# nverchev/PointCloudCounterfactual

Measured on AMD Instinct MI355X. Metric: clouds/sec Chamfer+EMD fwd+bwd, N=2048 B=32, higher is better.
Workload: dtype f32; 1 GPU; BASELINE configs[1]+[2]: N=2048 B=32 per GPU, nn_distance (Chamfer, mean) fwd+bwd + match_cost (approxmatch+matchcost) fwd+bwd through the autograd surface; inputs = "recon" clouds (reference permuted + N(0, 0.02^2): a trained autoencoder, SURVEY 8(d)); the 8(d) stress set (both clouds i.i.d. U[0,1]^3) is value_stress (--full); emd_mode=implicit, batch_per_gpu=32, n_points=2048, global_batch=32, parallelism=batch-sharded x1, no data-path collective, launcher=single process

## Files before the change

pointcloudcounterfactual_amd/backend.py:

```python

from __future__ import annotations

import ctypes

import torch

from pointcloudcounterfactual_amd import _lib
from pointcloudcounterfactual_amd._lib import call, ptr

_L = _lib.lib
F32, I32 = torch.float32, torch.int32


def _sizes(set_d: torch.Tensor, set_q: torch.Tensor) -> tuple[int, int, int]:
    return set_d.size(0), set_d.size(1), set_q.size(1)


def ApproxMatch(set_d: torch.Tensor, set_q: torch.Tensor) -> list[torch.Tensor]:
    b, n, m = _sizes(set_d, set_q)
    dev = set_d.device
    match = torch.empty((b, m, n), dtype=torch.float32, device=dev)
    temp = torch.empty((b, (n + m) * 2), dtype=torch.float32, device=dev)
    call(_L.pcc_approxmatch, 'ApproxMatch', dev, b, n, m, ptr(set_d, 'set_d', F32, dev), ptr(set_q, 'set_q', F32, dev),
         ptr(match, 'match', F32, dev), ptr(temp, 'temp', F32, dev))
    return [match, temp]


def ApproxMatchCost(set_d: torch.Tensor, set_q: torch.Tensor) -> list[torch.Tensor]:
    b, n, m = _sizes(set_d, set_q)
    dev = set_d.device
    match = torch.empty((b, m, n), dtype=torch.float32, device=dev)
    temp = torch.empty((b, (n + m) * 2), dtype=torch.float32, device=dev)
    cost = torch.empty((b,), dtype=torch.float32, device=dev)
    call(_L.pcc_approxmatch_cost, 'ApproxMatchCost', dev, b, n, m, ptr(set_d, 'set_d', F32, dev),
         ptr(set_q, 'set_q', F32, dev), ptr(match, 'match', F32, dev), ptr(temp, 'temp', F32, dev),
         ptr(cost, 'cost', F32, dev))
    return [match, temp, cost]


def MatchCostImplicit(set_d: torch.Tensor, set_q: torch.Tensor, with_grad: bool) -> list[torch.Tensor]:
    b, n, m = _sizes(set_d, set_q)
    dev = set_d.device
    cost = torch.empty((b,), dtype=torch.float32, device=dev)
    out = [cost]
    g1 = g2 = None
    if with_grad:
        g1 = torch.empty((b, n, 3), dtype=torch.float32, device=dev)
        g2 = torch.empty((b, m, 3), dtype=torch.float32, device=dev)
        out += [g1, g2]
    call(_L.pcc_match_cost, 'MatchCostImplicit', dev, b, n, m, ptr(set_d, 'set_d', F32, dev),
         ptr(set_q, 'set_q', F32, dev), None, ptr(cost, 'cost', F32, dev), ptr(g1, 'grad1', F32, dev),
         ptr(g2, 'grad2', F32, dev))
    return out


def MatchCost(set_d: torch.Tensor, set_q: torch.Tensor, match: torch.Tensor) -> torch.Tensor:
    b, n, m = _sizes(set_d, set_q)
    dev = set_d.device
    out = torch.empty((b,), dtype=torch.float32, device=dev)
    if match.numel() != b * n * m:
        raise RuntimeError(f'match has {match.numel()} elements, expected {b}x{m}x{n}')
    call(_L.pcc_matchcost, 'MatchCost', dev, b, n, m, ptr(set_d, 'set_d', F32, dev), ptr(set_q, 'set_q', F32, dev),
         ptr(match, 'match', F32, dev), ptr(out, 'cost', F32, dev))
    return out


def MatchCostGrad(set_d: torch.Tensor, set_q: torch.Tensor, match: torch.Tensor) -> list[torch.Tensor]:
    b, n, m = _sizes(set_d, set_q)
    dev = set_d.device
    grad1 = torch.empty((b, n, 3), dtype=torch.float32, device=dev)
    grad2 = torch.empty((b, m, 3), dtype=torch.float32, device=dev)
    if match.numel() != b * n * m:
        raise RuntimeError(f'match has {match.numel()} elements, expected {b}x{m}x{n}')
    call(_L.pcc_matchcostgrad, 'MatchCostGrad', dev, b, n, m, ptr(set_d, 'set_d', F32, dev),
         ptr(set_q, 'set_q', F32, dev), ptr(match, 'match', F32, dev), ptr(grad1, 'grad1', F32, dev),
         ptr(grad2, 'grad2', F32, dev))
    return [grad1, grad2]


def MatchCostGradScaled(set_d: torch.Tensor, set_q: torch.Tensor, match: torch.Tensor,
                        grad_cost: torch.Tensor) -> list[torch.Tensor]:
    b, n, m = _sizes(set_d, set_q)
    dev = set_d.device
    grad1 = torch.empty((b, n, 3), dtype=torch.float32, device=dev)
    grad2 = torch.empty((b, m, 3), dtype=torch.float32, device=dev)
    if match.numel() != b * n * m or grad_cost.numel() != b:
        raise RuntimeError('MatchCostGradScaled: match / grad_cost shapes do not match the clouds')
    call(_L.pcc_matchcostgrad_scaled, 'MatchCostGradScaled', dev, b, n, m, ptr(set_d, 'set_d', F32, dev),
         ptr(set_q, 'set_q', F32, dev), ptr(match, 'match', F32, dev), ptr(grad_cost, 'grad_cost', F32, dev),
         ptr(grad1, 'grad1', F32, dev), ptr(grad2, 'grad2', F32, dev))
    return [grad1, grad2]


def NNDistance(set_d: torch.Tensor, set_q: torch.Tensor) -> list[torch.Tensor]:
    b, n, m = _sizes(set_d, set_q)
    dev = set_d.device
    dist1 = torch.empty((b, n), dtype=torch.float32, device=dev)
    idx1 = torch.empty((b, n), dtype=torch.int32, device=dev)
    dist2 = torch.empty((b, m), dtype=torch.float32, device=dev)
    idx2 = torch.empty((b, m), dtype=torch.int32, device=dev)
    call(_L.pcc_nndistance, 'NNDistance', dev, b, n, ptr(set_d, 'set_d', F32, dev), m, ptr(set_q, 'set_q', F32, dev),
         ptr(dist1, 'dist1', F32, dev), ptr(idx1, 'idx1', I32, dev), ptr(dist2, 'dist2', F32, dev),
         ptr(idx2, 'idx2', I32, dev))
    return [dist1, idx1, dist2, idx2]


def ChamferLoss(set_d: torch.Tensor, set_q: torch.Tensor, mean: bool) -> list[torch.Tensor]:
    b, n, m = _sizes(set_d, set_q)
    dev = set_d.device
    loss = torch.empty((b,), dtype=torch.float32, device=dev)
    dist1 = torch.empty((b, n), dtype=torch.float32, device=dev)
    idx1 = torch.empty((b, n), dtype=torch.int32, device=dev)
    dist2 = torch.empty((b, m), dtype=torch.float32, device=dev)
    idx2 = torch.empty((b, m), dtype=torch.int32, device=dev)
    call(_L.pcc_chamfer_loss, 'ChamferLoss', dev, b, n, ptr(set_d, 'set_d', F32, dev), m, ptr(set_q, 'set_q', F32, dev),
         int(mean), ptr(loss, 'loss', F32, dev), ptr(dist1, 'dist1', F32, dev), ptr(idx1, 'idx1', I32, dev),
         ptr(dist2, 'dist2', F32, dev), ptr(idx2, 'idx2', I32, dev))
    return [loss, dist1, idx1, dist2, idx2]


def ChamferLossGrad(set_d: torch.Tensor, set_q: torch.Tensor, idx1: torch.Tensor, idx2: torch.Tensor,
                    grad_loss: torch.Tensor, mean: bool) -> list[torch.Tensor]:
    b, n, m = _sizes(set_d, set_q)
    dev = set_d.device
    grad1 = torch.empty((b, n, 3), dtype=torch.float32, device=dev)
    grad2 = torch.empty((b, m, 3), dtype=torch.float32, device=dev)
    if idx1.numel() != b * n or idx2.numel() != b * m or grad_loss.numel() != b:
        raise RuntimeError('ChamferLossGrad: idx / grad_loss shapes do not match the clouds')
    grad_loss, stride = _batch_stride(grad_loss, b)
    call(_L.pcc_chamfer_loss_grad, 'ChamferLossGrad', dev, b, n, ptr(set_d, 'set_d', F32, dev), m,
         ptr(set_q, 'set_q', F32, dev), ptr(idx1, 'idx1', I32, dev), ptr(idx2, 'idx2', I32, dev),
         ptr(grad_loss, 'grad_loss', F32, dev), stride, int(mean), ptr(grad1, 'grad1', F32, dev),
         ptr(grad2, 'grad2', F32, dev))
    return [grad1, grad2]


def ChamferEMD(set_d: torch.Tensor, set_q: torch.Tensor, mean: bool, with_grad: bool,
               return_dist: bool = False) -> list[torch.Tensor]:
    b, n, m = _sizes(set_d, set_q)
    dev = set_d.device
    loss = torch.empty((b,), dtype=torch.float32, device=dev)
    idx1 = torch.empty((b, n), dtype=torch.int32, device=dev)
    idx2 = torch.empty((b, m), dtype=torch.int32, device=dev)
    cost = torch.empty((b,), dtype=torch.float32, device=dev)
    out = [loss, idx1, idx2, cost]
    g1 = g2 = None
    if with_grad:
        g1 = torch.empty((b, n, 3), dtype=torch.float32, device=dev)
        g2 = torch.empty((b, m, 3), dtype=torch.float32, device=dev)
        out += [g1, g2]
    d1 = torch.empty((b, n), dtype=torch.float32, device=dev)
    d2 = torch.empty((b, m), dtype=torch.float32, device=dev)
    call(_L.pcc_chamfer_emd, 'ChamferEMD', dev, b, n, ptr(set_d, 'set_d', F32, dev), m, ptr(set_q, 'set_q', F32, dev),
         int(mean), ptr(loss, 'loss', F32, dev), ptr(d1, 'dist1', F32, dev), ptr(idx1, 'idx1', I32, dev),
         ptr(d2, 'dist2', F32, dev), ptr(idx2, 'idx2', I32, dev), ptr(cost, 'cost', F32, dev),
         ptr(g1, 'emd_grad1', F32, dev), ptr(g2, 'emd_grad2', F32, dev))
    if return_dist:
        out += [d1, d2]
    return out


def _batch_stride(g: torch.Tensor, b: int) -> tuple[torch.Tensor, int]:
    stride = g.stride(0) if g.dim() == 1 and b > 1 else 1
    if stride == 0:
        return g[:1], 0
    if stride != 1:
        return g.contiguous(), 1
    return g, 1


def ChamferEMDGrad(set_d: torch.Tensor, set_q: torch.Tensor, idx1: torch.Tensor, idx2: torch.Tensor,
                   grad_chamfer: torch.Tensor, mean: bool, emd_grad1: torch.Tensor, emd_grad2: torch.Tensor,
                   grad_emd: torch.Tensor) -> list[torch.Tensor]:
    b, n, m = _sizes(set_d, set_q)
    dev = set_d.device
    grad1 = torch.empty((b, n, 3), dtype=torch.float32, device=dev)
    grad2 = torch.empty((b, m, 3), dtype=torch.float32, device=dev)
    if (idx1.numel() != b * n or idx2.numel() != b * m or grad_chamfer.numel() != b or grad_emd.numel() != b
            or emd_grad1.numel() != b * n * 3 or emd_grad2.numel() != b * m * 3):
        raise RuntimeError('ChamferEMDGrad: shapes do not match the clouds')
    grad_chamfer, sc = _batch_stride(grad_chamfer, b)
    grad_emd, se = _batch_stride(grad_emd, b)
    call(_L.pcc_chamfer_emd_grad, 'ChamferEMDGrad', dev, b, n, ptr(set_d, 'set_d', F32, dev), m,
         ptr(set_q, 'set_q', F32, dev), ptr(idx1, 'idx1', I32, dev), ptr(idx2, 'idx2', I32, dev),
         ptr(grad_chamfer, 'grad_chamfer', F32, dev), sc, int(mean), ptr(emd_grad1, 'emd_grad1', F32, dev),
         ptr(emd_grad2, 'emd_grad2', F32, dev), ptr(grad_emd, 'grad_emd', F32, dev), se, ptr(grad1, 'grad1', F32, dev),
         ptr(grad2, 'grad2', F32, dev))
    return [grad1, grad2]


def NNDistanceGrad(set_d: torch.Tensor, set_q: torch.Tensor, idx1: torch.Tensor, idx2: torch.Tensor,
                   grad_dist1: torch.Tensor, grad_dist2: torch.Tensor) -> list[torch.Tensor]:
    b, n, m = _sizes(set_d, set_q)
    dev = set_d.device
    grad1 = torch.empty((b, n, 3), dtype=torch.float32, device=dev)
    grad2 = torch.empty((b, m, 3), dtype=torch.float32, device=dev)
    if idx1.numel() != b * n or grad_dist1.numel() != b * n or idx2.numel() != b * m or grad_dist2.numel() != b * m:
        raise RuntimeError('NNDistanceGrad: idx/grad_dist shapes do not match the clouds')
    call(_L.pcc_nndistancegrad, 'NNDistanceGrad', dev, b, n, ptr(set_d, 'set_d', F32, dev), m,
         ptr(set_q, 'set_q', F32, dev), ptr(grad_dist1, 'grad_dist1', F32, dev), ptr(idx1, 'idx1', I32, dev),
         ptr(grad_dist2, 'grad_dist2', F32, dev), ptr(idx2, 'idx2', I32, dev), ptr(grad1, 'grad1', F32, dev),
         ptr(grad2, 'grad2', F32, dev))
    return [grad1, grad2]


def SlicedWasserstein(set_d: torch.Tensor, set_q: torch.Tensor, theta: torch.Tensor, grad1: bool = False, grad2: bool = False,
                      per_direction: bool = False) -> list[torch.Tensor | None]:
    if set_d.dim() != 3 or set_d.size(2) != 3 or set_q.shape != set_d.shape:
        raise ValueError(f'SlicedWasserstein: clouds must be [B,N,3] of one shape, got {tuple(set_d.shape)} and {tuple(set_q.shape)}')
    if theta.dim() != 2 or theta.size(1) != 3:
        raise ValueError(f'SlicedWasserstein: directions must be [P,3], got {tuple(theta.shape)}')
    b, n, p = set_d.size(0), set_d.size(1), theta.size(0)
    dev = set_d.device
    cost = torch.empty((b,), dtype=torch.float32, device=dev)
    cost_p = torch.empty((b, p), dtype=torch.float32, device=dev) if per_direction else None
    g1 = torch.empty((b, n, 3), dtype=torch.float32, device=dev) if grad1 else None
    g2 = torch.empty((b, n, 3), dtype=torch.float32, device=dev) if grad2 else None
    call(_L.pcc_sliced_wasserstein, 'SlicedWasserstein', dev, b, n, p, ptr(set_d, 'set_d', F32, dev), ptr(set_q, 'set_q', F32, dev),
         ptr(theta, 'directions', F32, dev), ptr(cost, 'cost', F32, dev), ptr(cost_p, 'cost_p', F32, dev),
         ptr(g1, 'grad1', F32, dev), ptr(g2, 'grad2', F32, dev))
    return [cost, cost_p, g1, g2]


def Sinkhorn(set_d: torch.Tensor, set_q: torch.Tensor, eps: list[float], debias: bool = True, grad1: bool = False,
             grad2: bool = False, potentials: bool = False) -> list[torch.Tensor | None]:
    if set_d.dim() != 3 or set_q.dim() != 3 or set_d.size(2) != 3 or set_q.size(2) != 3 or set_d.size(0) != set_q.size(0):
        raise ValueError(f'Sinkhorn: clouds must be [B,N,3] and [B,M,3], got {tuple(set_d.shape)} and {tuple(set_q.shape)}')
    b, n, m = _sizes(set_d, set_q)
    dev = set_d.device
    sched = (ctypes.c_float * len(eps))(*eps)
    cost = torch.empty((b,), dtype=torch.float32, device=dev)
    p1 = torch.empty((b, n), dtype=torch.float32, device=dev) if potentials else None
    p2 = torch.empty((b, m), dtype=torch.float32, device=dev) if potentials else None
    g1 = torch.empty((b, n, 3), dtype=torch.float32, device=dev) if grad1 else None
    g2 = torch.empty((b, m, 3), dtype=torch.float32, device=dev) if grad2 else None
    call(_L.pcc_sinkhorn, 'Sinkhorn', dev, b, n, m, ptr(set_d, 'set_d', F32, dev), ptr(set_q, 'set_q', F32, dev), len(eps),
         ctypes.cast(sched, ctypes.c_void_p), int(bool(debias)), ptr(cost, 'cost', F32, dev), ptr(p1, 'pot1', F32, dev),
         ptr(p2, 'pot2', F32, dev), ptr(g1, 'grad1', F32, dev), ptr(g2, 'grad2', F32, dev))
    return [cost, p1, p2, g1, g2]
```

pointcloudcounterfactual_amd/csrc/am_pair.hip:

```cpp
#include "approxmatch.hpp"
#include "wave_ops.hpp"

#include <algorithm>

namespace {

using pcc::sq3;

constexpr int kPairRB = 8;
constexpr int kPairPad = 65;

struct PairArgs {
    int n, m, n4, m4;
    const float *soa1, *soa2;
    const float *lv;
    LevelConsts lc;
    float cut2[kLevels];
    float *cost_part;
    float *part1;
    float *part2;
    int col_blocks, row_tiles, bc;
};

template <int Q, bool GRAD>
__global__ __launch_bounds__(256) void am_pair_kernel(PairArgs a) {
    __shared__ float4 lds_l[kPairRT][3];
    __shared__ int lds_mask[kPairRT];
    __shared__ float stash[GRAD ? 4 * kPairRB * 3 * kPairPad : 4];
    __shared__ float lds_red[4];
    const int tid = threadIdx.x, lane = tid & 63;
    const int w = __builtin_amdgcn_readfirstlane(tid >> 6);
    const int cbn = a.col_blocks, rtn = a.row_tiles;
    const int item = (int)blockIdx.x / a.bc, smp = (int)blockIdx.x - item * a.bc;
    const int shift_k = item / cbn, cblk = item - shift_k * cbn;
    const int base_r = (int)(((long long)(2 * cblk + 1) * rtn) / (2 * cbn));
    const int shift = ((shift_k + 1) >> 1) * ((shift_k & 1) ? 1 : -1);
    const int rtile = ((base_r + shift) % rtn + rtn) % rtn;
    const int l0 = rtile * kPairRT;
    const int kb = cblk * 64 * Q;
    const int k0 = kb + lane * Q;
    const size_t nm4 = (size_t)a.n4 + a.m4;
    const float *lvb = a.lv + (size_t)smp * kLevels * nm4;
    const float *s1 = a.soa1 + (size_t)smp * 3 * a.n4;
    const float *s2 = a.soa2 + (size_t)smp * 3 * a.m4;
    const int lcnt = min(kPairRT, a.m - l0);

    float rowx = 0.f, rowy = 0.f, rowz = 0.f, rowr[kLevels];
#pragma unroll
    for (int i = 0; i < kLevels; i++) rowr[i] = 0.f;
    if (tid < lcnt) {
        const int l = l0 + tid;
        rowx = s2[l];
        rowy = s2[a.m4 + l];
        rowz = s2[2 * a.m4 + l];
#pragma unroll
        for (int i = 0; i < kLevels; i++) rowr[i] = lvb[(size_t)i * nm4 + a.n4 + l];
    }
    float x1[Q], y1[Q], z1[Q], rl[kLevels][Q];
    float blo[3] = {__builtin_inff(), __builtin_inff(), __builtin_inff()};
    float bhi[3] = {-__builtin_inff(), -__builtin_inff(), -__builtin_inff()};
#pragma unroll
    for (int q = 0; q < Q; q++) {
        const bool real = k0 + q < a.n;
        const int k = real ? k0 + q : a.n - 1;
        x1[q] = s1[k];
        y1[q] = s1[a.n4 + k];
        z1[q] = s1[2 * a.n4 + k];
#pragma unroll
        for (int i = 0; i < kLevels; i++) rl[i][q] = real ? lvb[(size_t)i * nm4 + k] : 0.f;
        blo[0] = fminf(blo[0], x1[q]); bhi[0] = fmaxf(bhi[0], x1[q]);
        blo[1] = fminf(blo[1], y1[q]); bhi[1] = fmaxf(bhi[1], y1[q]);
        blo[2] = fminf(blo[2], z1[q]); bhi[2] = fmaxf(bhi[2], z1[q]);
    }
#pragma unroll
    for (int c = 0; c < 3; c++) {
#pragma unroll
        for (int off = 1; off < 64; off <<= 1) {
            blo[c] = fminf(blo[c], __shfl_xor(blo[c], off, 64));
            bhi[c] = fmaxf(bhi[c], __shfl_xor(bhi[c], off, 64));
        }
    }
    if (tid < lcnt) {
        const float bx = fmaxf(fmaxf(blo[0] - rowx, rowx - bhi[0]), 0.f);
        const float by = fmaxf(fmaxf(blo[1] - rowy, rowy - bhi[1]), 0.f);
        const float bz = fmaxf(fmaxf(blo[2] - rowz, rowz - bhi[2]), 0.f);
        const float bd2 = bx * bx + by * by + bz * bz;
        int mask = 0;
#pragma unroll
        for (int i = 0; i < kLevels; i++) mask |= (rowr[i] != 0.f && !(bd2 > a.cut2[i])) ? (1 << i) : 0;
        lds_l[tid][0] = make_float4(rowx, rowy, rowz, rowr[0]);
        lds_l[tid][1] = make_float4(rowr[1], rowr[2], rowr[3], rowr[4]);
        lds_l[tid][2] = make_float4(rowr[5], rowr[6], rowr[7], rowr[8]);
        lds_mask[tid] = mask;
    }
    float g1[Q][3];
#pragma unroll
    for (int q = 0; q < Q; q++) g1[q][0] = g1[q][1] = g1[q][2] = 0.f;
    float csum = 0.f;
    float *my_stash = stash + (GRAD ? w * kPairRB * 3 * kPairPad : 0);
    __syncthreads();

    for (int base = 0; base < lcnt; base += 4 * kPairRB) {
#pragma unroll 1
        for (int s = 0; s < kPairRB; s++) {
            const int li = base + 4 * s + w;
            float rx = 0.f, ry = 0.f, rz = 0.f;
            const int mask = li < lcnt ? __builtin_amdgcn_readfirstlane(lds_mask[li]) : 0;
            if (mask) {
                const float4 A = lds_l[li][0], B = lds_l[li][1], Cc = lds_l[li][2];
                const float rr[kLevels] = {A.w, B.x, B.y, B.z, B.w, Cc.x, Cc.y, Cc.z, Cc.w};
                float ex[Q], ey[Q], ez[Q], d[Q], acc[Q];
#pragma unroll
                for (int q = 0; q < Q; q++) {
                    ex[q] = A.x - x1[q];
                    ey[q] = A.y - y1[q];
                    ez[q] = A.z - z1[q];
                    d[q] = sq3(ex[q], ey[q], ez[q]);
                    acc[q] = 0.f;
                }
#pragma unroll
                for (int i = 0; i < kLevels; i++) {
                    if (mask & (1 << i)) {
#pragma unroll
                        for (int q = 0; q < Q; q++)
                            acc[q] = __builtin_fmaf(fast_exp2(a.lc.c[i] * d[q]) * rl[i][q], rr[i], acc[q]);
                    }
                }
#pragma unroll
                for (int q = 0; q < Q; q++) {
                    if (GRAD) {
                        float dm;
                        asm("v_max_f32 %0, %1, %2" : "=v"(dm) : "v"(d[q]), "v"(1e-20f));
                        const float f = acc[q] * __builtin_amdgcn_rsqf(dm);
                        csum = __builtin_fmaf(f, d[q], csum);
                        g1[q][0] = __builtin_fmaf(-ex[q], f, g1[q][0]);
                        g1[q][1] = __builtin_fmaf(-ey[q], f, g1[q][1]);
                        g1[q][2] = __builtin_fmaf(-ez[q], f, g1[q][2]);
                        rx = __builtin_fmaf(ex[q], f, rx);
                        ry = __builtin_fmaf(ey[q], f, ry);
                        rz = __builtin_fmaf(ez[q], f, rz);
                    } else {
                        csum = __builtin_fmaf(acc[q], __builtin_amdgcn_sqrtf(d[q]), csum);
                    }
                }
            }
            if (GRAD) {
                my_stash[(s * 3 + 0) * kPairPad + lane] = rx;
                my_stash[(s * 3 + 1) * kPairPad + lane] = ry;
                my_stash[(s * 3 + 2) * kPairPad + lane] = rz;
            }
        }
        if (GRAD) {
            const int v = lane % 24, h = lane / 24;
            float t = 0.f;
            __builtin_amdgcn_wave_barrier();
            if (lane < 48) {
                const float *src = my_stash + v * kPairPad + h * 32;
#pragma unroll 8
                for (int i = 0; i < 32; i++) t += src[i];
            }
            __builtin_amdgcn_wave_barrier();
            const float hi = __shfl(t, lane + 24, 64);
            const int sl = v / 3, c = v - sl * 3;
            const int li = base + 4 * sl + w;
            if (lane < 24 && li < lcnt)
                a.part2[(((size_t)smp * cbn + cblk) * a.m4 + (l0 + li)) * 3 + c] = t + hi;
        }
    }
    csum = pcc::wave_sum_down(csum);
    if (lane == 0) lds_red[w] = csum;
    __syncthreads();
    if (tid == 0)
        a.cost_part[(size_t)smp * cbn * rtn + rtile * cbn + cblk] =
            ((lds_red[0] + lds_red[1]) + lds_red[2]) + lds_red[3];
    if (GRAD) {
        static_assert(Q * 3 * 64 <= 4 * kPairRB * 3 * kPairPad, "column merge reuses the stash");
        for (int src = 1; src < 4; src++) {
            __syncthreads();
            if (w == src) {
#pragma unroll
                for (int q = 0; q < Q; q++)
#pragma unroll
                    for (int c = 0; c < 3; c++) stash[(q * 3 + c) * 64 + lane] = g1[q][c];
            }
            __syncthreads();
            if (w == 0) {
#pragma unroll
                for (int q = 0; q < Q; q++)
#pragma unroll
                    for (int c = 0; c < 3; c++) g1[q][c] += stash[(q * 3 + c) * 64 + lane];
            }
        }
        if (w == 0) {
            float *dst = a.part1 + (((size_t)smp * rtn + rtile) * a.n4) * 3;
#pragma unroll
            for (int q = 0; q < Q; q++) {
                if (k0 + q < a.n) {
#pragma unroll
                    for (int c = 0; c < 3; c++) dst[(size_t)(k0 + q) * 3 + c] = g1[q][c];
                }
            }
        }
    }
}

struct FinishArgs {
    int parts[3], npts[2], pitch[2];
    const float *part[3];
    const int *perm[2];
    const float *scale;
    float *out[3];
    const float *ch_d1, *ch_d2;
    float *ch_loss;
    int ch_n, ch_m, ch_mean;
    const int *flags;
};
__global__ __launch_bounds__(256) void pair_finish_kernel(FinishArgs f) {
    __shared__ float red[256];
    const int which = blockIdx.z, smp = blockIdx.y, tid = threadIdx.x;
    if (which == 3) {
        if (blockIdx.x) return;
        __shared__ float red2[256];
        float s1 = 0.f, s2 = 0.f;
        auto strided_sum = [&](const float *d, int cnt) -> float {
            float acc = 0.f;
            for (int i0 = tid; i0 < cnt; i0 += 8 * 256) {
                float v[8];
#pragma unroll
                for (int u = 0; u < 8; u++) v[u] = d[min(i0 + u * 256, cnt - 1)];
#pragma unroll
                for (int u = 0; u < 8; u++)
                    if (i0 + u * 256 < cnt) acc += v[u];
            }
            return acc;
        };
        s1 = strided_sum(f.ch_d1 + (size_t)smp * f.ch_n, f.ch_n);
        s2 = strided_sum(f.ch_d2 + (size_t)smp * f.ch_m, f.ch_m);
        red[tid] = s1;
        red2[tid] = s2;
        __syncthreads();
        for (int off = 128; off > 0; off >>= 1) {
            if (tid < off) {
                red[tid] += red[tid + off];
                red2[tid] += red2[tid + off];
            }
            __syncthreads();
        }
        if (tid == 0) f.ch_loss[smp] = f.ch_mean ? red2[0] / (float)f.ch_m + red[0] / (float)f.ch_n : red[0] + red2[0];
        return;
    }
    const bool poisoned = f.flags && (f.flags[(size_t)smp * kLiveRow + kInfSlot] | f.flags[(size_t)smp * kLiveRow + kInfSlot + 1] |
                                      f.flags[(size_t)smp * kLiveRow + kErrSlot]);
    if (which == 2) {
        if (blockIdx.x) return;
        const int parts = f.parts[2];
        float s = 0.f;
        for (int i = tid; i < parts; i += 256) s += f.part[2][(size_t)smp * parts + i];
        red[tid] = s;
        __syncthreads();
        for (int off = 128; off > 0; off >>= 1) {
            if (tid < off) red[tid] += red[tid + off];
            __syncthreads();
        }
        if (tid == 0) f.out[2][smp] = poisoned ? __builtin_nanf("") : red[0];
        return;
    }
    if (!f.out[which]) return;
    const int npts = f.npts[which], pitch = f.pitch[which], parts = f.parts[which];
    const int i = blockIdx.x * 256 + tid;
    if (i >= npts * 3) return;
    const int s = i / 3, c = i - s * 3;
    const float *p = f.part[which] + (size_t)smp * parts * pitch * 3 + i;
    const int pt = f.perm[which][(size_t)smp * npts + s];
    const size_t stride = (size_t)pitch * 3;
    float acc = p[0];
    int t = 1;
    for (; t + 8 <= parts; t += 8) {
        float v[8];
#pragma unroll
        for (int u = 0; u < 8; u++) v[u] = p[(size_t)(t + u) * stride];
#pragma unroll
        for (int u = 0; u < 8; u++) acc += v[u];
    }
    {
        float v[7];
#pragma unroll
        for (int u = 0; u < 7; u++) v[u] = p[(size_t)min(t + u, parts - 1) * stride];
#pragma unroll
        for (int u = 0; u < 7; u++)
            if (t + u < parts) acc += v[u];
    }
    f.out[which][((size_t)smp * npts + pt) * 3 + c] = poisoned ? __builtin_nanf("") : f.scale ? acc * f.scale[smp] : acc;
}

template <int Q>
int launch_pair(const PairArgs &pa, dim3 grid, bool grad, hipStream_t st) {
    pcc::ProfScope prof(grad ? "am_pair_kernel<grad>" : "am_pair_kernel<cost>", st);
    if (grad) hipLaunchKernelGGL((am_pair_kernel<Q, true>), grid, dim3(256), 0, st, pa);
    else hipLaunchKernelGGL((am_pair_kernel<Q, false>), grid, dim3(256), 0, st, pa);
    return pcc::check_launch("match_cost(pair)");
}

}

namespace pcc {

int launch_pair_finish(const AmDims &L, const WsView &v, int s0, int bc, int col_blocks, int row_tiles, const float *grad_cost,
                       float *cost, float *grad1, float *grad2, const ChamferOut *chamfer, hipStream_t lst) {
    const size_t o = (size_t)s0;
    const int n = L.n, m = L.m;
    const bool grad = grad1 && grad2;
    const LevelConsts lc = make_levels();
    PairArgs pa{};
    pa.n = n; pa.m = m; pa.n4 = L.n4; pa.m4 = L.m4;
    pa.soa1 = v.soa1; pa.soa2 = v.soa2; pa.lv = v.lv;
    pa.lc = lc;
    for (int i = 0; i < kLevels; i++) pa.cut2[i] = zero_cut2(lc, i);
    pa.cost_part = v.pair_cost;
    pa.part1 = grad ? v.part1 : nullptr;
    pa.part2 = grad ? v.part2 : nullptr;
    pa.col_blocks = col_blocks; pa.row_tiles = row_tiles; pa.bc = bc;
    if ((long long)col_blocks * row_tiles * bc > 0x7fffffffLL) return pcc::invalid("match_cost: grid too large");
    const dim3 grid((unsigned)(col_blocks * row_tiles * bc));
    if (int rc = launch_pair<kPairQ>(pa, grid, grad, lst)) return rc;
    FinishArgs f{};
    f.parts[0] = row_tiles; f.parts[1] = col_blocks; f.parts[2] = col_blocks * row_tiles;
    f.npts[0] = n; f.npts[1] = m; f.pitch[0] = L.n4; f.pitch[1] = L.m4;
    f.part[0] = pa.part1; f.part[1] = pa.part2; f.part[2] = pa.cost_part;
    f.perm[0] = v.perm1; f.perm[1] = v.perm2;
    f.scale = grad_cost ? grad_cost + o : nullptr;
    f.out[0] = grad ? grad1 + o * n * 3 : nullptr;
    f.out[1] = grad ? grad2 + o * m * 3 : nullptr;
    f.out[2] = cost + o;
    f.flags = v.live_cnt;
    if (chamfer) {
        f.ch_d1 = chamfer->dist1 + o * n; f.ch_d2 = chamfer->dist2 + o * m; f.ch_loss = chamfer->loss + o;
        f.ch_n = n; f.ch_m = m; f.ch_mean = chamfer->mean;
    }
    {
        pcc::ProfScope prof("pair_finish_kernel", lst);
        const int blocks = grad ? pcc::ceil_div(std::max(n, m) * 3, 256) : 1;
        hipLaunchKernelGGL(pair_finish_kernel, dim3(blocks, bc, chamfer ? 4 : 3), dim3(256), 0, lst, f);
    }
    return pcc::check_launch("match_cost(reduce)");
}
}
```

pointcloudcounterfactual_amd/csrc/approxmatch.hip:

```cpp
#include "approxmatch.hpp"
#include "pcc_test_hooks.h"
#include "wave_ops.hpp"

#include <algorithm>
#include <functional>
#include <mutex>
#include <type_traits>

namespace {

using pcc::sq3;
using pcc::WsView;

enum Phase { PH_A = 0, PH_B = 1, PH_CA = 2, PH_C = 3 };

__device__ __forceinline__ float pass_a_ratio(float remL, float sum) { return remL / (1e-9f + sum); }
struct PassB {
    float ratio, remain;
};
__device__ __forceinline__ PassB pass_b(float remR, float sum) {
    const float sumr = sum * remR;
    const float consumption = __builtin_fminf(remR / (sumr + 1e-9f), 1.0f);
    return {consumption * remR, __builtin_fmaxf(0.0f, remR - sumr)};
}
__device__ __forceinline__ float pass_c_left(float remL, float ratioL, float sum) { return __builtin_fmaxf(0.0f, remL - ratioL * sum); }

struct PhaseArgs {
    int n_own, n_cand, tiles, batch;
    int own_n4, cand_n4, own_nb, cand_nb;
    const float *own_soa, *cand_soa;
    const float *cand_box;
    const float *own_box16;
    const float *w0, *w1;
    long long w0_stride, w1_stride;
    float w0c;
    float c0, c1;
    float cut2;
    float cut2_fine;
    int first;
    int level;
    float multiL, multiR;
    float *remain;
    float *remain_out;
    long long remain_stride;
    const float *ratio_in;
    float *ratio_out;
    long long ratio_stride;
    float *clist;
    int *clist_cnt;
    int cl_n4;
    const unsigned *mask_in;
    unsigned *mask_out;
    int mask_words;
    const int *live_in;
    int *live_out;
};

enum Var { V_PLAIN = 0, V_CULL = 1, V_COWN = 3, V_CLIST = 4 };

struct Sched {
    int n, m, n4, m4, nb1, nb2;
    const float *soa1, *soa2, *box1, *box2;
    float *rem, *lv;
    float multiL, multiR;
    float *clist;
    int *clist_cnt;
    int *live_cnt;
    unsigned *live_mask;
    int skip;
    LevelConsts lc;
};

inline int sched_phases() { return 2 * kLevels + 1; }

inline PhaseArgs build_phase(const Sched &sc, int p, int *mode_out, int *var_out) {
    const long long nm4 = (long long)sc.n4 + sc.m4;
    const long long rs = (long long)sc.n4 + 2LL * sc.m4;
    PhaseArgs a{};
    a.multiL = sc.multiL;
    a.multiR = sc.multiR;
    const bool set1_owns = (p == 0) || (p % 2 == 0);
    if (set1_owns) {
        a.n_own = sc.n; a.n_cand = sc.m; a.own_n4 = sc.n4; a.cand_n4 = sc.m4; a.own_nb = sc.nb1; a.cand_nb = sc.nb2;
        a.own_soa = sc.soa1; a.cand_soa = sc.soa2; a.cand_box = sc.box2;
        a.own_box16 = sc.box1;
    } else {
        a.n_own = sc.m; a.n_cand = sc.n; a.own_n4 = sc.m4; a.cand_n4 = sc.n4; a.own_nb = sc.nb2; a.cand_nb = sc.nb1;
        a.own_soa = sc.soa2; a.cand_soa = sc.soa1; a.cand_box = sc.box1;
        a.own_box16 = sc.box2;
    }
    int mode, var;
    if (p == 0) {
        mode = PH_A;
        var = sc.skip ? V_CULL : V_PLAIN;
        a.level = 0;
        a.w0 = nullptr; a.w0c = sc.multiR; a.c0 = sc.lc.c[0]; a.first = 1;
        a.cut2 = zero_cut2(sc.lc, 0);
        a.ratio_out = sc.lv; a.ratio_stride = kLevels * nm4;
    } else {
        const int i = (p - 1) / 2;
        float *ratioL = sc.lv + (size_t)i * nm4, *ratioR = ratioL + sc.n4;
        a.level = i;
        a.first = (i == 0);
        a.c0 = sc.lc.c[i];
        if (p % 2 == 1) {
            mode = PH_B;
            var = !sc.skip ? V_PLAIN : i <= 2 ? V_CULL : V_COWN;
            a.w0 = ratioL; a.w0_stride = kLevels * nm4;
            a.cut2 = zero_cut2(sc.lc, i);
            a.remain = sc.rem + sc.n4 + (i & 1) * sc.m4;
            a.remain_out = sc.rem + sc.n4 + ((i + 1) & 1) * sc.m4;
            a.remain_stride = rs;
            a.ratio_out = ratioR; a.ratio_stride = kLevels * nm4;
            if (var == V_COWN) { a.clist = sc.clist; a.clist_cnt = sc.clist_cnt; a.cl_n4 = sc.m4; }
            if (sc.live_mask) {
                const int words = mask_words(sc.m4);
                a.mask_words = words;
                if (i + 1 < kLevels && (var == V_COWN || i == 2)) a.mask_out = sc.live_mask + (size_t)(i + 1) * words;
                if (var == V_COWN) {
                    a.mask_in = sc.live_mask + (size_t)i * words;
                    a.remain = a.remain_out = sc.rem + sc.n4 + sc.m4;
                }
            }
            if (sc.live_cnt) {
                a.live_in = (var == V_COWN && i >= 1) ? sc.live_cnt + i : nullptr;
                a.live_out = i + 1 < kLevels ? sc.live_cnt + i + 1 : nullptr;
            }
        } else {
            mode = i + 1 < kLevels ? PH_CA : PH_C;
            var = !sc.skip ? V_PLAIN : i <= 2 ? V_CULL : V_CLIST;
            if (var == V_CLIST) { a.clist = sc.clist; a.clist_cnt = sc.clist_cnt; a.cl_n4 = sc.m4; }
            a.w0 = ratioR; a.w0_stride = kLevels * nm4;
            a.w1 = sc.rem + sc.n4 + ((i + 1) & 1) * sc.m4; a.w1_stride = rs;
            a.remain = sc.rem; a.remain_stride = rs;
            a.ratio_in = ratioL; a.ratio_stride = kLevels * nm4;
            const int lc_i = i + 1 < kLevels ? i + 1 : i;
            a.cut2 = zero_cut2(sc.lc, lc_i);
            a.cut2_fine = zero_cut2(sc.lc, i);
            if (i + 1 < kLevels) {
                a.c1 = sc.lc.c[i + 1];
                a.ratio_out = sc.lv + (size_t)(i + 1) * nm4;
            }
        }
    }
    *mode_out = mode;
    *var_out = var;
    return a;
}

template <int NW, int R, int S, int CH>
struct PhaseLds {
    static constexpr int kC = (3 + NW) * CH;
    static constexpr int kRed = NW * S * 64 * R;
    static constexpr int kOwn = 64 * R;
    static constexpr int kWave = S;
    static constexpr int floats = kC + kRed + kOwn + kWave + 4;
};

template <int MODE, int R, int S, int CH, int VAR, int G = 1>
__device__ __forceinline__ void am_phase_body(const PhaseArgs &a, int smp, int tile, float *smem) {
    constexpr int T = 64 * S;
    constexpr int TQ = 64 * R / G;
    constexpr int PQ = 64 * R;
    static_assert(G == 1 || (VAR == V_COWN && R == 1), "lane-split owners: owner-compacted launches only");
    constexpr int NW = (MODE == PH_CA) ? 2 : 1;
    constexpr bool W0_CONST = (MODE == PH_A);
    constexpr bool COWN = VAR == V_COWN, CLIST = VAR == V_CLIST;
    static_assert(VAR == V_PLAIN || COWN || CLIST, "the box-culled passes run on am_fine_kernel");
    static_assert(!(CLIST && W0_CONST), "pass A of the first level has constant weights");
    static_assert(TQ <= T, "one epilogue owner per thread");
    using L = PhaseLds<NW, R, S, CH>;
    float *lds_c = smem;
    float *red = smem + L::kC;
    int *own_idx = reinterpret_cast<int *>(red + L::kRed);
    int *wave_cnt = own_idx + L::kOwn;

    const int tid = threadIdx.x;
    const int lane = tid & 63;
    const int w = __builtin_amdgcn_readfirstlane(tid >> 6);
    const int sub = G > 1 ? lane / TQ : 0;
    const float *O = a.own_soa + (size_t)smp * 3 * a.own_n4;
    const float *C = a.cand_soa + (size_t)smp * 3 * a.cand_n4;
    const float *W0 = W0_CONST ? nullptr : a.w0 + (size_t)smp * a.w0_stride;
    const float *W1 = (NW == 2) ? a.w1 + (size_t)smp * a.w1_stride : nullptr;

    if (!COWN && tile * TQ >= a.n_own) return;
    static_assert(CH / 4 <= T, "one float4 group per thread and chunk");
    float4 st_x, st_y, st_z, st_0, st_1;
    auto stage_load = [&](const float *Cc, const float *W0c, const float *W1c, int pitch, int q0, int ngroups) {
        const int i = min(tid, max(ngroups - 1, 0));
        st_x = reinterpret_cast<const float4 *>(Cc + q0)[i];
        st_y = reinterpret_cast<const float4 *>(Cc + (size_t)pitch + q0)[i];
        st_z = reinterpret_cast<const float4 *>(Cc + (size_t)2 * pitch + q0)[i];
        st_0 = make_float4(a.w0c, a.w0c, a.w0c, a.w0c);
        st_1 = st_0;
        if (!W0_CONST) st_0 = *reinterpret_cast<const float4 *>(W0c + q0 + 4 * i);
        if (NW == 2) st_1 = *reinterpret_cast<const float4 *>(W1c + q0 + 4 * i);
    };
    if (COWN) stage_load(C, W0, W1, a.cand_n4, 0, (min(CH, a.n_cand) + 3) / 4);
    int n_valid = min(TQ, a.n_own - tile * TQ);
    if (COWN) {
        const int lo = tile * TQ, hi = lo + TQ;
        const unsigned *mk = a.mask_in + (size_t)smp * kLevels * a.mask_words;
        unsigned *mnext = (tile == 0 && a.mask_out) ? a.mask_out + (size_t)smp * kLevels * a.mask_words : nullptr;
        const int wpt = (a.mask_words + T - 1) / T;
        unsigned word = 0;
        int mine = 0;
        if (wpt == 1) {
            word = mk[min(tid, a.mask_words - 1)];
            word &= -(unsigned)(tid < a.mask_words);
            if (mnext && tid < a.mask_words) atomicAnd(&mnext[tid], word);
            mine = __popc(word);
        } else {
            for (int j = tid * wpt; j < min(tid * wpt + wpt, a.mask_words); j++) {
                const unsigned wj = mk[j];
                if (mnext) atomicAnd(&mnext[j], wj);
                mine += __popc(wj);
            }
        }
        int incl = mine;
#pragma unroll
        for (int off = 1; off < 64; off <<= 1) {
            const int v = __shfl_up(incl, off, 64);
            incl += lane >= off ? v : 0;
        }
        if (lane == 63) wave_cnt[w] = incl;
        __syncthreads();
        int before = 0, total = 0;
#pragma unroll
        for (int i = 0; i < S; i++) {
            const int c = __builtin_amdgcn_readfirstlane(wave_cnt[i]);
            before += i < w ? c : 0;
            total += c;
        }
        int pos = before + incl - mine - lo;
        auto deal = [&](unsigned bits, int first_owner) {
            while (bits) {
                const int bit = __builtin_ctz(bits);
                bits &= bits - 1;
                if ((unsigned)pos < (unsigned)TQ) own_idx[pos] = first_owner + bit;
                pos++;
            }
        };
        if (wpt == 1) {
            deal(word, tid * 32);
        } else {
            for (int j = tid * wpt; j < min(tid * wpt + wpt, a.mask_words); j++) deal(mk[j], j * 32);
        }
        if (a.clist_cnt && tile == 0 && tid == 0) a.clist_cnt[smp] = total;
        n_valid = min(TQ, total - lo);
        if (n_valid <= 0) return;
        (void)hi;
        __syncthreads();
    }
    int own_e = -1;
    if (tid < TQ && tid < n_valid) own_e = COWN ? own_idx[tid] : tile * TQ + tid;

    float ox[R], oy[R], oz[R], s0[R], s1[R];
    float t0x = 0.f, t1x = 0.f;
#pragma unroll
    for (int r = 0; r < R; r++) {
        const int e = G > 1 ? (lane & (TQ - 1)) : r * 64 + lane;
        int o = COWN ? own_idx[e < n_valid ? e : 0] : tile * TQ + e;
        o = o < a.n_own ? o : a.n_own - 1;
        ox[r] = O[o];
        oy[r] = O[a.own_n4 + o];
        oz[r] = O[2 * a.own_n4 + o];
        s0[r] = 0.f;
        s1[r] = 0.f;
    }
    float pre_rem = 0.f, pre_ratio = 0.f;
    {
        const int oe = max(own_e, 0);
        if (MODE != PH_A && !a.first) pre_rem = a.remain[(size_t)smp * a.remain_stride + oe];
        if (MODE == PH_CA || MODE == PH_C) pre_ratio = a.ratio_in[(size_t)smp * a.ratio_stride + oe];
    }
    const float4 *X4 = reinterpret_cast<const float4 *>(lds_c);
    const float4 *Y4 = X4 + CH / 4;
    const float4 *Z4 = Y4 + CH / 4;
    const float4 *A4 = Z4 + CH / 4;
    const float4 *B4 = A4 + CH / 4;
    const float c0 = a.c0, c1 = a.c1;

    const int n_cand = CLIST ? __builtin_amdgcn_readfirstlane(a.clist_cnt[smp]) : a.n_cand;
    if (CLIST) {
        C = a.clist + (size_t)smp * 5 * a.cl_n4;
        W0 = C + (size_t)3 * a.cl_n4;
        W1 = C + (size_t)4 * a.cl_n4;
    }
    const int cand_pitch = CLIST ? a.cl_n4 : a.cand_n4;
    for (int q0 = 0; q0 < n_cand; q0 += CH) {
        const int cnt = min(CH, n_cand - q0);
        int ngroups = (cnt + 3) / 4;
        if (q0) __syncthreads();
        {
            float4 *dst4 = reinterpret_cast<float4 *>(lds_c);
            if (!(COWN && q0 == 0)) stage_load(C, W0, W1, cand_pitch, q0, ngroups);
            const int i = tid;
            if (i < ngroups) {
                float4 vx = st_x, vy = st_y, vz = st_z, v0 = st_0, v1 = st_1;
                if (CLIST && i * 4 + 3 >= cnt) {
                    vx.y = i * 4 + 1 < cnt ? vx.y : 0.f; vx.z = i * 4 + 2 < cnt ? vx.z : 0.f; vx.w = 0.f;
                    vy.y = i * 4 + 1 < cnt ? vy.y : 0.f; vy.z = i * 4 + 2 < cnt ? vy.z : 0.f; vy.w = 0.f;
                    vz.y = i * 4 + 1 < cnt ? vz.y : 0.f; vz.z = i * 4 + 2 < cnt ? vz.z : 0.f; vz.w = 0.f;
                }
                if ((W0_CONST || CLIST) && i * 4 + 3 >= cnt) {
                    v0.x = i * 4 + 0 < cnt ? v0.x : 0.f;
                    v0.y = i * 4 + 1 < cnt ? v0.y : 0.f;
                    v0.z = i * 4 + 2 < cnt ? v0.z : 0.f;
                    v0.w = 0.f;
                    if (NW == 2) {
                        v1.x = i * 4 + 0 < cnt ? v1.x : 0.f;
                        v1.y = i * 4 + 1 < cnt ? v1.y : 0.f;
                        v1.z = i * 4 + 2 < cnt ? v1.z : 0.f;
                        v1.w = 0.f;
                    }
                }
                dst4[i] = vx;
                dst4[CH / 4 + i] = vy;
                dst4[2 * (CH / 4) + i] = vz;
                dst4[3 * (CH / 4) + i] = v0;
                if (NW == 2) dst4[4 * (CH / 4) + i] = v1;
            }
        }
        const int nblk = (ngroups + 3) / 4;
        __syncthreads();
        for (int blk = w; blk < nblk; blk += S) {
            const int g_end = min(blk * 4 + 4, ngroups);
            for (int g = blk * 4 + sub; g < g_end; g += G) {
                const float4 x = X4[g], y = Y4[g], z = Z4[g], wa = A4[g];
                float4 wb;
                if (NW == 2) wb = B4[g];
#pragma unroll
                for (int r = 0; r < R; r++) {
                    const float d0 = sq3(x.x - ox[r], y.x - oy[r], z.x - oz[r]);
                    const float d1 = sq3(x.y - ox[r], y.y - oy[r], z.y - oz[r]);
                    const float d2 = sq3(x.z - ox[r], y.z - oy[r], z.z - oz[r]);
                    const float d3 = sq3(x.w - ox[r], y.w - oy[r], z.w - oz[r]);
                    if (R == 1) {
                        s0[r] = __builtin_fmaf(fast_exp2(c0 * d0), wa.x, s0[r]);
                        t0x = __builtin_fmaf(fast_exp2(c0 * d1), wa.y, t0x);
                        s0[r] = __builtin_fmaf(fast_exp2(c0 * d2), wa.z, s0[r]);
                        t0x = __builtin_fmaf(fast_exp2(c0 * d3), wa.w, t0x);
                        if (NW == 2) {
                            s1[r] = __builtin_fmaf(fast_exp2(c1 * d0), wb.x, s1[r]);
                            t1x = __builtin_fmaf(fast_exp2(c1 * d1), wb.y, t1x);
                            s1[r] = __builtin_fmaf(fast_exp2(c1 * d2), wb.z, s1[r]);
                            t1x = __builtin_fmaf(fast_exp2(c1 * d3), wb.w, t1x);
                        }
                    } else {
                        s0[r] = __builtin_fmaf(fast_exp2(c0 * d0), wa.x, s0[r]);
                        s0[r] = __builtin_fmaf(fast_exp2(c0 * d1), wa.y, s0[r]);
                        s0[r] = __builtin_fmaf(fast_exp2(c0 * d2), wa.z, s0[r]);
                        s0[r] = __builtin_fmaf(fast_exp2(c0 * d3), wa.w, s0[r]);
                        if (NW == 2) {
                            s1[r] = __builtin_fmaf(fast_exp2(c1 * d0), wb.x, s1[r]);
                            s1[r] = __builtin_fmaf(fast_exp2(c1 * d1), wb.y, s1[r]);
                            s1[r] = __builtin_fmaf(fast_exp2(c1 * d2), wb.z, s1[r]);
                            s1[r] = __builtin_fmaf(fast_exp2(c1 * d3), wb.w, s1[r]);
                        }
                    }
                }
            }
        }
    }
    if (R == 1) {
        s0[0] += t0x;
        s1[0] += t1x;
    }
    if (G > 1) {
        s0[0] += __shfl_xor(s0[0], TQ, 64);
        if (G == 4) s0[0] += __shfl_xor(s0[0], 2 * TQ, 64);
    }
#pragma unroll
    for (int r = 0; r < R; r++) {
        red[(0 * S + w) * PQ + r * 64 + lane] = s0[r];
        if (NW == 2) red[(1 * S + w) * PQ + r * 64 + lane] = s1[r];
    }
    __syncthreads();
    if (own_e < 0) return;
    {
        const int e = tid;
        const int o = own_e;
        float t0 = red[e], t1 = 0.f;
        if (NW == 2) t1 = red[(1 * S) * PQ + e];
#pragma unroll
        for (int s = 1; s < S; s++) {
            t0 += red[(0 * S + s) * PQ + e];
            if (NW == 2) t1 += red[(1 * S + s) * PQ + e];
        }
        if (MODE == PH_A) {
            a.ratio_out[(size_t)smp * a.ratio_stride + o] = pass_a_ratio(a.multiL, t0);
        } else if (MODE == PH_B) {
            const PassB pb = pass_b(a.first ? a.multiR : pre_rem, t0);
            const float ratio_new = pb.ratio, remain_new = pb.remain;
            a.ratio_out[(size_t)smp * a.ratio_stride + o] = ratio_new;
            a.remain_out[(size_t)smp * a.remain_stride + o] = remain_new;
            if (a.live_out) {
                const unsigned long long alive = __ballot(remain_new != 0.f);
                if (lane == 0) atomicAdd(&a.live_out[(size_t)smp * kLiveRow], (int)__popcll(alive));
            }
            if (COWN && a.mask_out && remain_new == 0.f)
                atomicAnd(&a.mask_out[(size_t)smp * kLevels * a.mask_words + (o >> 5)], ~(1u << (o & 31)));
            if (COWN && a.clist) {
                float cx = ox[0], cy = oy[0], cz = oz[0];
#pragma unroll
                for (int r = 1; r < R; r++) {
                    cx = w == r ? ox[r] : cx;
                    cy = w == r ? oy[r] : cy;
                    cz = w == r ? oz[r] : cz;
                }
                float *cl = a.clist + (size_t)smp * 5 * a.cl_n4 + tile * TQ + e;
                cl[0] = cx;
                cl[(size_t)a.cl_n4] = cy;
                cl[(size_t)2 * a.cl_n4] = cz;
                cl[(size_t)3 * a.cl_n4] = ratio_new;
                cl[(size_t)4 * a.cl_n4] = remain_new;
            }
        } else {
            const float left = pass_c_left(a.first ? a.multiL : pre_rem, pre_ratio, t0);
            a.remain[(size_t)smp * a.remain_stride + o] = left;
            if (MODE == PH_CA) a.ratio_out[(size_t)smp * a.ratio_stride + o] = pass_a_ratio(left, t1);
        }
    }
}

template <int MODE, int R, int S, int CH, int VAR, int G = 1>
__global__ __launch_bounds__(64 * S) void am_phase_kernel(PhaseArgs a) {
    __shared__ __attribute__((aligned(16))) float smem[PhaseLds<(MODE == PH_CA ? 2 : 1), R, S, CH>::floats];
    constexpr bool COWN = VAR == V_COWN;
    int smp, tile;
    const int bid = (int)blockIdx.x, nwg = (int)gridDim.x;
    if (COWN) {
        if (a.batch % 8 == 0) {
            const int per = a.batch / 8, i = bid / 8;
            smp = (bid % 8) + 8 * (i % per);
            tile = i / per;
        } else {
            smp = bid % a.batch;
            tile = bid / a.batch;
        }
        if (a.live_in && tile > 0 && tile * (64 * R / G) >= a.live_in[(size_t)smp * kLiveRow]) return;
    } else {
        const int lid = pcc::xcd_contiguous(bid, nwg);
        smp = lid / a.tiles;
        tile = lid - smp * a.tiles;
    }
    am_phase_body<MODE, R, S, CH, VAR, G>(a, smp, tile, smem);
}

constexpr int kFineS = 8;
constexpr int kFineOG = 16;
constexpr int kFineGroups = 64 / kFineOG;
constexpr int kFineQ = 4;

struct FineOwners {
    float x[kFineQ], y[kFineQ], z[kFineQ];
};
struct FineRows {
    const float *x, *y, *z, *w0, *w1;
};

__device__ __forceinline__ void fine_group_box(const float *own_box, int own_nb, int smp, int g16, float4 &lo, float4 &hi) {
    lo = make_float4(__builtin_inff(), __builtin_inff(), __builtin_inff(), 0.f);
    hi = make_float4(-__builtin_inff(), -__builtin_inff(), -__builtin_inff(), 0.f);
    if (g16 < own_nb) {
        const float4 *ob = reinterpret_cast<const float4 *>(own_box + ((size_t)smp * own_nb + g16) * 8);
        lo = ob[0];
        hi = ob[1];
    }
}

__device__ __forceinline__ float fine_box_d2(const float4 &glo, const float4 &ghi, const float *cand_box) {
    const float4 *cb = reinterpret_cast<const float4 *>(cand_box);
    const float4 lo = cb[0], hi = cb[1];
    const float dx = fmaxf(fmaxf(glo.x - hi.x, lo.x - ghi.x), 0.f);
    const float dy = fmaxf(fmaxf(glo.y - hi.y, lo.y - ghi.y), 0.f);
    const float dz = fmaxf(fmaxf(glo.z - hi.z, lo.z - ghi.z), 0.f);
    return dx * dx + dy * dy + dz * dz;
}

template <int NBLK>
__device__ __forceinline__ void fine_block_list(bool keep, bool outer_only, int tid, int tg, int tb, int w, int lane,
                                                int *wave_cnt, unsigned char (*items)[NBLK], unsigned char *need) {
    if (tid < NBLK) need[tid] = 0;
    const unsigned long long bal = __ballot(keep);
    if (lane == 0) wave_cnt[w] = __popcll(bal);
    __syncthreads();
    const int before = (w & 1) ? wave_cnt[w - 1] : 0;
    if (keep) {
        items[tg][before + __popcll(bal & ((1ull << lane) - 1ull))] = (unsigned char)(tb | (outer_only ? 128 : 0));
        need[tb] = 1;
    }
    __syncthreads();
}

template <int NW>
__device__ __forceinline__ void fine_walk(const FineRows &rows, const unsigned char *list, int nitems, int cs, int cl, float c0,
                                          float c1, const FineOwners &own, float (&s0)[kFineQ], float (&s1)[kFineQ]) {
    for (int it = cs; it < nitems; it += 2) {
        const int item = __builtin_amdgcn_readfirstlane((int)list[it]);
        const int ci = (item & 127) * kBox + cl;
        const float x = rows.x[ci], y = rows.y[ci], z = rows.z[ci];
        if (NW == 2 && (item & 128)) {
            const float wb = rows.w1[ci];
#pragma unroll
            for (int j = 0; j < kFineQ; j++) s1[j] = __builtin_fmaf(fast_exp2(c1 * sq3(x - own.x[j], y - own.y[j], z - own.z[j])), wb, s1[j]);
            continue;
        }
        const float wa = rows.w0[ci];
        float wb = 0.f;
        if (NW == 2) wb = rows.w1[ci];
#pragma unroll
        for (int j = 0; j < kFineQ; j++) {
            const float d = sq3(x - own.x[j], y - own.y[j], z - own.z[j]);
            s0[j] = __builtin_fmaf(fast_exp2(c0 * d), wa, s0[j]);
            if (NW == 2) s1[j] = __builtin_fmaf(fast_exp2(c1 * d), wb, s1[j]);
        }
    }
}

template <int NW>
__device__ __forceinline__ void fine_reduce(float (&s0)[kFineQ], float (&s1)[kFineQ], float (*red)[2][64], int cs, int cl, int og, int quad) {
    const auto add = [](float a, float b) { return a + b; };
#pragma unroll
    for (int j = 0; j < kFineQ; j++) {
        s0[j] = pcc::row_reduce16(s0[j], add);
        if (NW == 2) s1[j] = pcc::row_reduce16(s1[j], add);
    }
    if (cl == 0) {
#pragma unroll
        for (int j = 0; j < kFineQ; j++) {
            red[0][cs][og * kFineOG + quad * kFineQ + j] = s0[j];
            if (NW == 2) red[1][cs][og * kFineOG + quad * kFineQ + j] = s1[j];
        }
    }
}

template <int MODE, int CH>
__global__ __launch_bounds__(64 * kFineS, MODE == PH_CA ? 4 : 8) void am_fine_kernel(PhaseArgs a) {
    constexpr int T = 64 * kFineS;
    constexpr int NW = (MODE == PH_CA) ? 2 : 1;
    constexpr bool W0_CONST = (MODE == PH_A);
    constexpr int NBLK = CH / kBox;
    static_assert(kFineGroups * NBLK == T, "one (owner group, candidate block) box test per thread");
    static_assert(kFineOG == kBox && kFineOG * kFineQ == 64, "a wave = 16 candidates x 4 owner quads");
    __shared__ __attribute__((aligned(16))) float lds_c[(3 + NW) * CH];
    __shared__ float red[NW][2][64];
    __shared__ unsigned char items[kFineGroups][NBLK];
    __shared__ unsigned char need[NBLK];
    __shared__ int wave_cnt[kFineS];

    const int lid = pcc::xcd_contiguous((int)blockIdx.x, (int)gridDim.x);
    const int smp = lid / a.tiles;
    const int tile = lid - smp * a.tiles;
    const int tid = threadIdx.x, lane = tid & 63;
    const int w = __builtin_amdgcn_readfirstlane(tid >> 6);
    const int og = w & (kFineGroups - 1);
    const int cs = w / kFineGroups;
    const int cl = lane & (kBox - 1);
    const int quad = lane / kBox;
    const float *O = a.own_soa + (size_t)smp * 3 * a.own_n4;
    const float *C = a.cand_soa + (size_t)smp * 3 * a.cand_n4;
    const float *W0 = W0_CONST ? nullptr : a.w0 + (size_t)smp * a.w0_stride;
    const float *W1 = (NW == 2) ? a.w1 + (size_t)smp * a.w1_stride : nullptr;

    FineOwners own;
    float s0[kFineQ], s1[kFineQ];
#pragma unroll
    for (int j = 0; j < kFineQ; j++) {
        int o = tile * 64 + og * kFineOG + quad * kFineQ + j;
        o = o < a.n_own ? o : a.n_own - 1;
        own.x[j] = O[o];
        own.y[j] = O[a.own_n4 + o];
        own.z[j] = O[2 * a.own_n4 + o];
        s0[j] = 0.f;
        s1[j] = 0.f;
    }
    const int own_e = (tid < 64 && tile * 64 + tid < a.n_own) ? tile * 64 + tid : -1;
    float pre_rem = 0.f, pre_ratio = 0.f;
    {
        const int oe = max(own_e, 0);
        if (MODE != PH_A && !a.first) pre_rem = a.remain[(size_t)smp * a.remain_stride + oe];
        if (MODE == PH_CA || MODE == PH_C) pre_ratio = a.ratio_in[(size_t)smp * a.ratio_stride + oe];
    }
    const int tg = tid / NBLK, tb = tid - tg * NBLK;
    float4 glo, ghi;
    fine_group_box(a.own_box16, a.own_nb, smp, tile * kFineGroups + tg, glo, ghi);
    const float c0 = a.c0, c1 = a.c1, cut2 = a.cut2;
    const FineRows rows = {lds_c, lds_c + CH, lds_c + 2 * CH, lds_c + 3 * CH, lds_c + 4 * CH};

    for (int q0 = 0; q0 < a.n_cand; q0 += CH) {
        const int cnt = min(CH, a.n_cand - q0);
        const int ngroups = (cnt + 3) / 4;
        const int nblk = (ngroups + 3) / 4;
        if (q0) __syncthreads();
        bool keep = false, outer_only = false;
        if (tb < nblk) {
            const float bd2 = fine_box_d2(glo, ghi, a.cand_box + ((size_t)smp * a.cand_nb + q0 / kBox + tb) * 8);
            keep = !(bd2 > cut2);
            outer_only = NW == 2 && bd2 > a.cut2_fine;
        }
        fine_block_list<NBLK>(keep, outer_only, tid, tg, tb, w, lane, wave_cnt, items, need);
        {
            float4 *dst4 = reinterpret_cast<float4 *>(lds_c);
            const float4 *sx = reinterpret_cast<const float4 *>(C + q0);
            const float4 *sy = reinterpret_cast<const float4 *>(C + (size_t)a.cand_n4 + q0);
            const float4 *sz = reinterpret_cast<const float4 *>(C + (size_t)2 * a.cand_n4 + q0);
            static_assert(CH / 4 <= T, "one float4 group per thread and chunk");
            const int i = tid;
            if (i < nblk * 4 && need[i >> 2]) {
                float4 vx = make_float4(0.f, 0.f, 0.f, 0.f), vy = vx, vz = vx, v0 = vx, v1 = vx;
                if (i < ngroups) {
                    vx = sx[i]; vy = sy[i]; vz = sz[i];
                    v0 = W0_CONST ? make_float4(a.w0c, a.w0c, a.w0c, a.w0c) : *reinterpret_cast<const float4 *>(W0 + q0 + 4 * i);
                    if (NW == 2) v1 = *reinterpret_cast<const float4 *>(W1 + q0 + 4 * i);
                    if (W0_CONST && i * 4 + 3 >= cnt) {
                        v0.x = i * 4 + 0 < cnt ? v0.x : 0.f;
                        v0.y = i * 4 + 1 < cnt ? v0.y : 0.f;
                        v0.z = i * 4 + 2 < cnt ? v0.z : 0.f;
                        v0.w = 0.f;
                    }
                }
                dst4[i] = vx;
                dst4[CH / 4 + i] = vy;
                dst4[2 * (CH / 4) + i] = vz;
                dst4[3 * (CH / 4) + i] = v0;
                if (NW == 2) dst4[4 * (CH / 4) + i] = v1;
            }
        }
        __syncthreads();
        fine_walk<NW>(rows, items[og], wave_cnt[2 * og] + wave_cnt[2 * og + 1], cs, cl, c0, c1, own, s0, s1);
    }
    fine_reduce<NW>(s0, s1, red, cs, cl, og, quad);
    __syncthreads();
    if (own_e < 0) return;
    const float sum0 = red[0][0][tid] + red[0][1][tid];
    const float sum1 = NW == 2 ? red[NW - 1][0][tid] + red[NW - 1][1][tid] : 0.f;
    if (MODE == PH_A) {
        a.ratio_out[(size_t)smp * a.ratio_stride + own_e] = pass_a_ratio(a.multiL, sum0);
    } else if (MODE == PH_B) {
        const PassB pb = pass_b(a.first ? a.multiR : pre_rem, sum0);
        a.ratio_out[(size_t)smp * a.ratio_stride + own_e] = pb.ratio;
        a.remain_out[(size_t)smp * a.remain_stride + own_e] = pb.remain;
        if (a.live_out) {
            const unsigned long long alive = __ballot(pb.remain != 0.f);
            if (lane == 0) atomicAdd(&a.live_out[(size_t)smp * kLiveRow], (int)__popcll(alive));
            if (a.mask_out && lane == 0) {
                unsigned *mo = a.mask_out + (size_t)smp * kLevels * a.mask_words;
                if (2 * tile < a.mask_words) mo[2 * tile] = (unsigned)alive;
                if (2 * tile + 1 < a.mask_words) mo[2 * tile + 1] = (unsigned)(alive >> 32);
            }
        }
    } else {
        const float left = pass_c_left(a.first ? a.multiL : pre_rem, pre_ratio, sum0);
        a.remain[(size_t)smp * a.remain_stride + own_e] = left;
        if (MODE == PH_CA) a.ratio_out[(size_t)smp * a.ratio_stride + own_e] = pass_a_ratio(left, sum1);
    }
}

constexpr int kFpPasses = 7;
constexpr int kFpCH = 2048;

struct FinePersistArgs {
    int n, m, n4, m4, nb1, nb2, tiles;
    const float *soa1, *soa2, *box1, *box2;
    float *rem, *lv;
    float multiL, multiR;
    float c[4], cut2[4];
    int *live_cnt;
    unsigned *live_mask;
    int mask_words;
    unsigned *host_err;
    int inject;
};

__global__ __launch_bounds__(64 * kFineS) void am_fine_persist_kernel(FinePersistArgs a) {
    constexpr int T = 64 * kFineS, CH = kFpCH, NBLK = CH / kBox;
    static_assert(kFineGroups * NBLK == T, "one (owner group, candidate block) box test per thread and direction");
    __shared__ __attribute__((aligned(16))) float lds_p[2][3 * CH];
    __shared__ __attribute__((aligned(16))) float lds_w[2][CH];
    __shared__ float red[2][2][64];
    __shared__ unsigned char items[kFineGroups][NBLK];
    __shared__ unsigned char need[NBLK];
    __shared__ int wave_cnt[kFineS];

    const int lid = pcc::xcd_contiguous((int)blockIdx.x, (int)gridDim.x);
    const int smp = lid / a.tiles;
    const int tile = lid - smp * a.tiles;
    const int tid = threadIdx.x, lane = tid & 63;
    const int w = __builtin_amdgcn_readfirstlane(tid >> 6);
    const int og = w & (kFineGroups - 1), cs = w / kFineGroups;
    const int cl = lane & (kBox - 1), quad = lane / kBox;
    const long long nm4 = (long long)a.n4 + a.m4, rs = (long long)a.n4 + 2LL * a.m4;
    const float *S1 = a.soa1 + (size_t)smp * 3 * a.n4;
    const float *S2 = a.soa2 + (size_t)smp * 3 * a.m4;
    float *LV = a.lv + (size_t)smp * kLevels * nm4;
    float *REM = a.rem + (size_t)smp * rs;
    int *row = a.live_cnt + (size_t)smp * kLiveRow;
    unsigned *bar = reinterpret_cast<unsigned *>(row + kBarSlot);
    unsigned *err = reinterpret_cast<unsigned *>(row + kErrSlot);

    for (int s = 0; s < 2; s++) {
        const float *S = s ? S2 : S1;
        const int p4 = s ? a.m4 : a.n4, ngroups = p4 / 4, nblk = (ngroups + 3) / 4;
        float4 *dst4 = reinterpret_cast<float4 *>(lds_p[s]);
        const float4 *sx = reinterpret_cast<const float4 *>(S);
        const float4 *sy = reinterpret_cast<const float4 *>(S + p4);
        const float4 *sz = reinterpret_cast<const float4 *>(S + 2 * (size_t)p4);
        for (int i = tid; i < nblk * 4; i += T) {
            float4 vx = make_float4(0.f, 0.f, 0.f, 0.f), vy = vx, vz = vx;
            if (i < ngroups) { vx = sx[i]; vy = sy[i]; vz = sz[i]; }
            dst4[i] = vx;
            dst4[CH / 4 + i] = vy;
            dst4[2 * (CH / 4) + i] = vz;
        }
    }
    FineOwners set1, set2;
#pragma unroll
    for (int j = 0; j < kFineQ; j++) {
        const int o = tile * 64 + og * kFineOG + quad * kFineQ + j;
        const int o1 = min(o, a.n - 1), o2 = min(o, a.m - 1);
        set1.x[j] = S1[o1]; set1.y[j] = S1[a.n4 + o1]; set1.z[j] = S1[2 * a.n4 + o1];
        set2.x[j] = S2[o2]; set2.y[j] = S2[a.m4 + o2]; set2.z[j] = S2[2 * a.m4 + o2];
    }
    const int tg = tid / NBLK, tb = tid - tg * NBLK;
    auto box_d2 = [&](const float *own_box, int own_nb, const float *cand_box, int cand_nb) -> float {
        float4 glo, ghi;
        fine_group_box(own_box, own_nb, smp, tile * kFineGroups + tg, glo, ghi);
        if (tb >= cand_nb) return __builtin_inff();
        return fine_box_d2(glo, ghi, cand_box + ((size_t)smp * cand_nb + tb) * 8);
    };
    const float d2_role0 = box_d2(a.box1, a.nb1, a.box2, a.nb2);
    const float d2_role1 = box_d2(a.box2, a.nb2, a.box1, a.nb1);
    const int own1 = (tid < 64 && tile * 64 + tid < a.n) ? tile * 64 + tid : -1;
    const int own2 = (tid < 64 && tile * 64 + tid < a.m) ? tile * 64 + tid : -1;
    float remL = 0.f, ratL = 0.f, remR = 0.f;
    unsigned arrivals = 0;
    bool ok = true;

    auto pass = [&](auto mode_tag, int i) {
        constexpr int MODE = decltype(mode_tag)::value;
        constexpr int NW = MODE == PH_CA ? 2 : 1;
        constexpr int ROLE = MODE == PH_B ? 1 : 0;
        const int n_cand = ROLE ? a.n : a.m, cand_n4 = ROLE ? a.n4 : a.m4;
        const int nblk = (cand_n4 / 4 + 3) / 4;
        const float c0 = a.c[i], c1 = a.c[MODE == PH_CA ? i + 1 : i];
        const float cut2 = a.cut2[MODE == PH_CA ? i + 1 : i];
        const float *P = lds_p[ROLE ? 0 : 1];
        const float bd2 = ROLE ? d2_role1 : d2_role0;
        const bool keep = tb < nblk && !(bd2 > cut2);
        const bool outer_only = NW == 2 && bd2 > a.cut2[i];
        fine_block_list<NBLK>(keep, outer_only, tid, tg, tb, w, lane, wave_cnt, items, need);
        {
            const float *W0 = MODE == PH_A ? nullptr : MODE == PH_B ? LV + (size_t)i * nm4 : LV + (size_t)i * nm4 + a.n4;
            const float *W1 = MODE == PH_CA ? REM + a.n4 + (size_t)((i + 1) & 1) * a.m4 : nullptr;
            for (int idx = tid; idx < nblk * kBox; idx += T) {
                if (!need[idx >> 4]) continue;
                float v0, v1 = 0.f;
                if (MODE == PH_A) v0 = idx < n_cand ? a.multiR : 0.f;
                else v0 = idx < cand_n4 ? pcc::agent_ld(W0 + idx) : 0.f;
                if (NW == 2) v1 = idx < cand_n4 ? pcc::agent_ld(W1 + idx) : 0.f;
                lds_w[0][idx] = v0;
                if (NW == 2) lds_w[1][idx] = v1;
            }
        }
        __syncthreads();
        float s0[kFineQ], s1[kFineQ];
#pragma unroll
        for (int j = 0; j < kFineQ; j++) s0[j] = s1[j] = 0.f;
        const FineRows rows = {P, P + CH, P + 2 * CH, lds_w[0], lds_w[1]};
        fine_walk<NW>(rows, items[og], wave_cnt[2 * og] + wave_cnt[2 * og + 1], cs, cl, c0, c1, ROLE ? set2 : set1, s0, s1);
        fine_reduce<NW>(s0, s1, red, cs, cl, og, quad);
        __syncthreads();
        const int own_e = ROLE ? own2 : own1;
        if (own_e >= 0) {
            const float sum0 = red[0][0][tid] + red[0][1][tid];
            const float sum1 = NW == 2 ? red[1][0][tid] + red[1][1][tid] : 0.f;
            if (MODE == PH_A) {
                ratL = pass_a_ratio(a.multiL, sum0);
                pcc::agent_st(LV + own_e, ratL);
            } else if (MODE == PH_B) {
                const PassB pb = pass_b(i == 0 ? a.multiR : remR, sum0);
                pcc::agent_st(LV + (size_t)i * nm4 + a.n4 + own_e, pb.ratio);
                pcc::agent_st(REM + a.n4 + (size_t)((i + 1) & 1) * a.m4 + own_e, pb.remain);
                remR = pb.remain;
                if (i == 2) {
                    const unsigned long long alive = __ballot(pb.remain != 0.f);
                    if (lane == 0) {
                        atomicAdd(&row[3], (int)__popcll(alive));
                        unsigned *mo = a.live_mask + ((size_t)smp * kLevels + 3) * a.mask_words;
                        if (2 * tile < a.mask_words) mo[2 * tile] = (unsigned)alive;
                        if (2 * tile + 1 < a.mask_words) mo[2 * tile + 1] = (unsigned)(alive >> 32);
                    }
                }
            } else {
                remL = pass_c_left(i == 0 ? a.multiL : remL, ratL, sum0);
                pcc::agent_st(REM + own_e, remL);
                ratL = pass_a_ratio(remL, sum1);
                pcc::agent_st(LV + (size_t)(i + 1) * nm4 + own_e, ratL);
            }
        }
    };
    auto barrier = [&]() -> bool {
        arrivals += (unsigned)a.tiles;
        return pcc::coresident_barrier<1, (1u << 22)>(bar, arrivals, err, a.host_err, [&] {
            const unsigned seen = pcc::agent_ld(bar);
            return 1u | ((arrivals / (unsigned)a.tiles) << 4) | ((seen & 0xfffu) << 8) | ((unsigned)smp << 20);
        });
    };
    if (a.inject && tile == 0 && tid == 0) pcc::coresident_fail(err, a.host_err, 1u | ((unsigned)smp << 20));
    __syncthreads();
    pass(std::integral_constant<int, PH_A>{}, 0);
    for (int i = 0; i < 3 && ok; i++) {
        ok = barrier();
        if (!ok) break;
        pass(std::integral_constant<int, PH_B>{}, i);
        ok = barrier();
        if (!ok) break;
        pass(std::integral_constant<int, PH_CA>{}, i);
    }
}

__global__ __launch_bounds__(256) void am_unpermute_kernel(int n, int m, int n4, int m4,
                                                            const float *__restrict__ lv_sorted,
                                                            const float *__restrict__ rem_sorted,
                                                            const int *__restrict__ rank1,
                                                            const int *__restrict__ rank2,
                                                            const int *__restrict__ flags,
                                                            float *__restrict__ lv, float *__restrict__ temp) {
    const int smp = blockIdx.y;
    const int i = blockIdx.x * 256 + threadIdx.x;
    if (i >= n + m) return;
    const int s = i < n ? rank1[(size_t)smp * n + i] : n4 + rank2[(size_t)smp * m + (i - n)];
    const size_t nm = (size_t)n + m, nm4 = (size_t)n4 + m4;
    const float *src = lv_sorted + (size_t)smp * kLevels * nm4;
    float *dst = lv + (size_t)smp * kLevels * nm;
    const bool failed = flags[(size_t)smp * kLiveRow + kErrSlot] != 0;
    float last = 0.f;
#pragma unroll
    for (int l = 0; l < kLevels; l++) {
        last = failed ? __builtin_nanf("") : src[(size_t)l * nm4 + s];
        dst[(size_t)l * nm + i] = last;
    }
    float *tb = temp + (size_t)smp * 2 * nm;
    tb[i] = failed ? __builtin_nanf("") : rem_sorted[(size_t)smp * (nm4 + m4) + (i < n ? s : s + m4)];
    tb[nm + i] = last;
}

constexpr int kMatLT = 64;
constexpr int kMatKT = 256;

template <bool COST, bool VEC>
__global__ __launch_bounds__(256) void am_materialise_kernel(int n, int m, const float *__restrict__ xyz1,
                                                              const float *__restrict__ xyz2,
                                                              const float *__restrict__ lv, LevelConsts lc,
                                                              float *__restrict__ match,
                                                              float *__restrict__ cost_part) {
    __shared__ float4 lds_l[kMatLT][3];
    __shared__ float lds_red[4];
    const int tid = threadIdx.x, lane = tid & 63;
    const int w = __builtin_amdgcn_readfirstlane(tid >> 6);
    const int smp = blockIdx.z;
    const int l0 = blockIdx.y * kMatLT;
    const int k0 = blockIdx.x * kMatKT + lane * 4;
    const size_t lvs = (size_t)kLevels * (n + m);
    const float *lvb = lv + (size_t)smp * lvs;
    const float *p1 = xyz1 + (size_t)smp * n * 3;
    const float *p2 = xyz2 + (size_t)smp * m * 3;
    const int lcnt = min(kMatLT, m - l0);

    if (tid < lcnt) {
        const int l = l0 + tid;
        float rr[kLevels];
#pragma unroll
        for (int i = 0; i < kLevels; i++) rr[i] = lvb[(size_t)i * (n + m) + n + l];
        lds_l[tid][0] = make_float4(p2[l * 3 + 0], p2[l * 3 + 1], p2[l * 3 + 2], rr[0]);
        lds_l[tid][1] = make_float4(rr[1], rr[2], rr[3], rr[4]);
        lds_l[tid][2] = make_float4(rr[5], rr[6], rr[7], rr[8]);
    }
    float x1[4], y1[4], z1[4], rl[kLevels][4];
#pragma unroll
    for (int q = 0; q < 4; q++) {
        int k = k0 + q;
        k = k < n ? k : n - 1;
        x1[q] = p1[k * 3 + 0];
        y1[q] = p1[k * 3 + 1];
        z1[q] = p1[k * 3 + 2];
#pragma unroll
        for (int i = 0; i < kLevels; i++) rl[i][q] = lvb[(size_t)i * (n + m) + k];
    }
    __syncthreads();
    float csum = 0.f;
    for (int li = w; li < lcnt; li += 4) {
        const float4 A = lds_l[li][0], B = lds_l[li][1], Cc = lds_l[li][2];
        const float rr[kLevels] = {A.w, B.x, B.y, B.z, B.w, Cc.x, Cc.y, Cc.z, Cc.w};
        int live[kLevels];
#pragma unroll
        for (int i = 0; i < kLevels; i++) live[i] = __builtin_amdgcn_readfirstlane((int)(rr[i] != 0.f));
        float d[4], acc[4];
#pragma unroll
        for (int q = 0; q < 4; q++) {
            d[q] = sq3(A.x - x1[q], A.y - y1[q], A.z - z1[q]);
            acc[q] = 0.f;
        }
#pragma unroll
        for (int i = 0; i < kLevels; i++) {
            if (live[i]) {
#pragma unroll
                for (int q = 0; q < 4; q++) acc[q] += (fast_exp2(lc.c[i] * d[q]) * rl[i][q]) * rr[i];
            }
        }
        float out[4];
#pragma unroll
        for (int q = 0; q < 4; q++) {
            out[q] = acc[q];
            if (COST && k0 + q < n) csum = __builtin_fmaf(acc[q], __builtin_amdgcn_sqrtf(d[q]), csum);
        }
        float *row = match + ((size_t)smp * m + (l0 + li)) * n;
        if (VEC) {
            if (k0 + 3 < n) {
                v4f o4 = {out[0], out[1], out[2], out[3]};
                __builtin_nontemporal_store(o4, reinterpret_cast<v4f *>(row + k0));
            } else {
#pragma unroll
                for (int q = 0; q < 4; q++)
                    if (k0 + q < n) row[k0 + q] = out[q];
            }
        } else {
#pragma unroll
            for (int q = 0; q < 4; q++)
                if (k0 + q < n) row[k0 + q] = out[q];
        }
    }
    if (COST) {
        csum = pcc::wave_sum_down(csum);
        if (lane == 0) lds_red[w] = csum;
        __syncthreads();
        if (tid == 0)
            cost_part[(size_t)smp * gridDim.x * gridDim.y + blockIdx.y * gridDim.x + blockIdx.x] =
                ((lds_red[0] + lds_red[1]) + lds_red[2]) + lds_red[3];
    }
}

constexpr int kPhCH = 2048;
constexpr int kClistCH = 1024;

static bool cull_enabled() {
    return pcc::tuning(PCC_TUNE_AM_NOCULL) == 0;
}

template <int MODE>
const char *phase_name(int level, bool skipping) {
    static const char *const names[4][kLevels][2] = {
        {{"am_phase_kernel<A> L0 plain", "am_phase_kernel<A> L0 fine"}, {"", ""}, {"", ""}, {"", ""}, {"", ""},
         {"", ""}, {"", ""}, {"", ""}, {"", ""}},
        {{"am_phase_kernel<B> L0 plain", "am_phase_kernel<B> L0 fine"},
         {"am_phase_kernel<B> L1 plain", "am_phase_kernel<B> L1 fine"},
         {"am_phase_kernel<B> L2 plain", "am_phase_kernel<B> L2 fine"},
         {"am_phase_kernel<B> L3 plain", "am_phase_kernel<B> L3 own"},
         {"am_phase_kernel<B> L4 plain", "am_phase_kernel<B> L4 own"},
         {"am_phase_kernel<B> L5 plain", "am_phase_kernel<B> L5 own"},
         {"am_phase_kernel<B> L6 plain", "am_phase_kernel<B> L6 own"},
         {"am_phase_kernel<B> L7 plain", "am_phase_kernel<B> L7 own"},
         {"am_phase_kernel<B> L8 plain", "am_phase_kernel<B> L8 own"}},
        {{"am_phase_kernel<CA> L0 plain", "am_phase_kernel<CA> L0 fine"},
         {"am_phase_kernel<CA> L1 plain", "am_phase_kernel<CA> L1 fine"},
         {"am_phase_kernel<CA> L2 plain", "am_phase_kernel<CA> L2 fine"},
         {"am_phase_kernel<CA> L3 plain", "am_phase_kernel<CA> L3 list"},
         {"am_phase_kernel<CA> L4 plain", "am_phase_kernel<CA> L4 list"},
         {"am_phase_kernel<CA> L5 plain", "am_phase_kernel<CA> L5 list"},
         {"am_phase_kernel<CA> L6 plain", "am_phase_kernel<CA> L6 list"},
         {"am_phase_kernel<CA> L7 plain", "am_phase_kernel<CA> L7 list"}, {"", ""}},
        {{"", ""}, {"", ""}, {"", ""}, {"", ""}, {"", ""}, {"", ""}, {"", ""}, {"", ""},
         {"am_phase_kernel<C> L8 plain", "am_phase_kernel<C> L8 list"}}};
    return names[MODE][level][skipping];
}

template <int MODE, int R, int S, int G = 1>
int launch_phase_rs(PhaseArgs a, int b, int var, hipStream_t st, const char *what) {
    a.tiles = pcc::ceil_div(a.n_own, 64 * R / G);
    a.batch = b;
    const long long grid = (long long)b * a.tiles;
    if (grid > 0x7fffffffLL) return pcc::invalid("approxmatch: grid too large");
    {
        const bool skipping = (var == V_CLIST && (MODE == PH_CA || MODE == PH_C)) || (var == V_COWN && MODE == PH_B);
        pcc::ProfScope prof(phase_name<MODE>(a.level, skipping), st);
        const dim3 g((unsigned)grid), blk(64 * S);
        if (var == V_CLIST && (MODE == PH_CA || MODE == PH_C))
            hipLaunchKernelGGL((am_phase_kernel<(MODE == PH_CA || MODE == PH_C) ? MODE : PH_C, R, S, kClistCH, V_CLIST>), g, blk, 0, st, a);
        else if (var == V_COWN && MODE == PH_B)
            hipLaunchKernelGGL((am_phase_kernel<PH_B, (G > 1 ? 1 : R), S, kPhCH, V_COWN, G>), g, blk, 0, st, a);
        else hipLaunchKernelGGL((am_phase_kernel<MODE, R, S, kPhCH, V_PLAIN>), g, blk, 0, st, a);
    }
    return pcc::check_launch(what);
}

template <int MODE>
int launch_fine(PhaseArgs a, int b, hipStream_t st, const char *what) {
    a.tiles = pcc::ceil_div(a.n_own, 64);
    a.batch = b;
    const long long grid = (long long)b * a.tiles;
    if (grid > 0x7fffffffLL) return pcc::invalid("approxmatch: grid too large");
    {
        pcc::ProfScope prof(phase_name<MODE>(a.level, true), st);
        hipLaunchKernelGGL((am_fine_kernel<(MODE == PH_C ? PH_CA : MODE), kPhCH>), dim3((unsigned)grid), dim3(64 * kFineS), 0, st, a);
    }
    return pcc::check_launch(what);
}

template <int MODE>
int launch_phase(const PhaseArgs &a, int b, int var, hipStream_t st, const char *what) {
    if (var == V_CULL) return launch_fine<MODE>(a, b, st, what);
    if (var == V_COWN) {
        if (a.live_in && a.level >= 5) return launch_phase_rs<MODE, 1, 8, 4>(a, b, var, st, what);
        if (a.live_in && a.level >= 4) return launch_phase_rs<MODE, 1, 8, 2>(a, b, var, st, what);
        return launch_phase_rs<MODE, 1, 8>(a, b, var, st, what);
    }
    const long long owners = (long long)b * a.n_own;
    if (var == V_CLIST && owners < 4LL * 65536) return launch_phase_rs<MODE, 1, 8>(a, b, var, st, what);
    if (owners >= 4LL * 65536) return launch_phase_rs<MODE, 4, 8>(a, b, var, st, what);
    if (owners >= 32768) return launch_phase_rs<MODE, 2, 8>(a, b, var, st, what);
    return launch_phase_rs<MODE, 1, 8>(a, b, var, st, what);
}

size_t cost_parts(int n, int m) { return (size_t)pcc::ceil_div(n, kMatKT) * pcc::ceil_div(m, kMatLT); }

struct WsLayout : pcc::AmDims {
    int b;
    int col_blocks, row_tiles;
    bool grad;
    size_t total;
    WsLayout(int b_, int n_, int m_, int col_blocks_ = 0, int row_tiles_ = 0, bool grad_ = false)
        : AmDims(n_, m_), b(b_), col_blocks(col_blocks_), row_tiles(row_tiles_), grad(grad_) {
        WsView unused;
        total = carve(0, 0, unused);
    }
    WsView view(char *base, int s) const {
        WsView v;
        carve(reinterpret_cast<uintptr_t>(base), (size_t)s, v);
        return v;
    }

  private:
    size_t carve(uintptr_t base, size_t s, WsView &v) const {
        size_t o = 0;
        auto sec = [&](auto *&p, size_t per) {
            using T = std::remove_reference_t<decltype(*p)>;
            p = reinterpret_cast<T *>(base + o + s * per * sizeof(T));
            o = (o + (size_t)b * per * sizeof(T) + 15) & ~(size_t)15;
        };
        sec(v.soa1, 3 * (size_t)n4);
        sec(v.soa2, 3 * (size_t)m4);
        sec(v.rank1, n);
        sec(v.rank2, m);
        sec(v.perm1, n);
        sec(v.perm2, m);
        sec(v.box1, (size_t)nb1 * 8);
        sec(v.box2, (size_t)nb2 * 8);
        sec(v.rem, rem_floats());
        sec(v.lv, lv_floats());
        sec(v.lv_orig, kLevels * ((size_t)n + m));
        sec(v.cpart, cost_parts(n, m));
        sec(v.clist, 5 * (size_t)m4);
        sec(v.clist_cnt, 1);
        sec(v.live_cnt, kLiveRow);
        sec(v.live_mask, (size_t)kLevels * mask_words(m4));
        sec(v.aos1, n);
        sec(v.aos2, m);
        sec(v.pair_cost, (size_t)col_blocks * row_tiles);
        sec(v.part1, grad ? (size_t)row_tiles * n4 * 3 : 0);
        sec(v.part2, grad ? (size_t)col_blocks * m4 * 3 : 0);
        return o;
    }
};

constexpr int kMaxLanes = 2;
hipStream_t side_stream() {
    static std::mutex mu;
    static hipStream_t streams[64] = {};
    int dev = 0;
    if (hipGetDevice(&dev) != hipSuccess || dev < 0 || dev >= 64) return nullptr;
    std::lock_guard<std::mutex> lk(mu);
    if (!streams[dev]) {
        int least = 0, greatest = 0;
        if (hipDeviceGetStreamPriorityRange(&least, &greatest) != hipSuccess) {
            (void)hipGetLastError();
            least = greatest = 0;
        }
        if (hipStreamCreateWithPriority(&streams[dev], hipStreamNonBlocking, greatest) != hipSuccess) {
            (void)hipGetLastError();
            if (hipStreamCreateWithFlags(&streams[dev], hipStreamNonBlocking) != hipSuccess) {
                streams[dev] = nullptr;
                (void)hipGetLastError();
            }
        }
    }
    return streams[dev];
}

struct ForkJoin {
    hipStream_t main, side = nullptr;
    ForkJoin(hipStream_t m, bool fork) : main(m) {
        if (!fork) return;
        hipEvent_t ev;
        if (hipEventCreateWithFlags(&ev, hipEventDisableTiming) != hipSuccess) return;
        if (hipEventRecord(ev, main) == hipSuccess) {
            hipStream_t s = side_stream();
            if (s && hipStreamWaitEvent(s, ev, 0) == hipSuccess) side = s;
        }
        (void)hipEventDestroy(ev);
    }
    ~ForkJoin() {
        if (!side) return;
        hipEvent_t ev;
        if (hipEventCreateWithFlags(&ev, hipEventDisableTiming) != hipSuccess) {
            (void)hipStreamSynchronize(side);
            return;
        }
        (void)hipEventRecord(ev, side);
        (void)hipStreamWaitEvent(main, ev, 0);
        (void)hipEventDestroy(ev);
    }
};

static bool resident_enabled() {
    return pcc::tuning(PCC_TUNE_AM_NORESIDENT) == 0;
}
int launch_fine_resident(const Sched &sc, int bc, hipStream_t st) {
    if (!sc.skip || !sc.live_cnt || !sc.live_mask || !resident_enabled()) return -1;
    if (sc.n > kFpCH || sc.m > kFpCH || sc.n < 1 || sc.m < 1) return -1;
    const int tiles = pcc::ceil_div(std::max(sc.n, sc.m), 64);
    FinePersistArgs a{};
    a.n = sc.n; a.m = sc.m; a.n4 = sc.n4; a.m4 = sc.m4; a.nb1 = sc.nb1; a.nb2 = sc.nb2; a.tiles = tiles;
    a.soa1 = sc.soa1; a.soa2 = sc.soa2; a.box1 = sc.box1; a.box2 = sc.box2;
    a.rem = sc.rem; a.lv = sc.lv; a.multiL = sc.multiL; a.multiR = sc.multiR;
    for (int i = 0; i < 4; i++) {
        a.c[i] = sc.lc.c[i];
        a.cut2[i] = zero_cut2(sc.lc, i);
    }
    a.live_cnt = sc.live_cnt;
    a.live_mask = sc.live_mask;
    a.mask_words = mask_words(sc.m4);
    static const int per_cu = [] {
        int r = 0;
        const void *k = reinterpret_cast<const void *>(am_fine_persist_kernel);
        if (hipOccupancyMaxActiveBlocksPerMultiprocessor(&r, k, 64 * kFineS, 0) != hipSuccess) (void)hipGetLastError();
        return r;
    }();
    if (per_cu < 2 || (long long)bc * tiles > pcc::device_cus()) return -1;
    pcc::CoresidentGate gate(pcc::kFineResident, st);
    if (!gate.ok) return -1;
    a.host_err = gate.sticky;
    a.inject = gate.inject;
    {
        pcc::ProfScope prof("am_fine_persist_kernel", st);
        hipLaunchKernelGGL(am_fine_persist_kernel, dim3((unsigned)(bc * tiles)), dim3(64 * kFineS), 0, st, a);
    }
    return pcc::check_launch("approxmatch(resident fine levels)");
}

Sched lane_sched(const WsLayout &L, const WsView &v, const LevelConsts &lc) {
    Sched sc{};
    sc.n = L.n; sc.m = L.m; sc.n4 = L.n4; sc.m4 = L.m4; sc.nb1 = L.nb1; sc.nb2 = L.nb2;
    sc.soa1 = v.soa1; sc.soa2 = v.soa2; sc.box1 = v.box1; sc.box2 = v.box2; sc.rem = v.rem; sc.lv = v.lv;
    if (L.n >= L.m) { sc.multiL = 1; sc.multiR = (float)(L.n / L.m); }
    else { sc.multiL = (float)(L.m / L.n); sc.multiR = 1; }
    sc.skip = cull_enabled() ? 1 : 0;
    sc.lc = lc;
    sc.clist = v.clist; sc.clist_cnt = v.clist_cnt;
    if (sc.skip) { sc.live_cnt = v.live_cnt; sc.live_mask = v.live_mask; }
    return sc;
}

int run_levels(const WsLayout &L, char *base, const float *xyz1, const float *xyz2, const LevelConsts &lc, hipStream_t st,
               const std::function<int(int, int, hipStream_t)> &lane_tail = nullptr,
               const std::function<int(int, int, hipStream_t)> &after_sort = nullptr) {
    if (const unsigned fw = pcc::take_coresident_failure(pcc::kFineResident)) {
        char buf[320];
        std::snprintf(buf, sizeof buf, "approxmatch: an earlier call on this device did not complete (a sample barrier of the resident "
                      "fine-level launch timed out: barrier %u of sample %u saw %u arrivals; the implicit path reported NaN for those "
                      "samples); this call was not started", (fw >> 4) & 0xfu, fw >> 20, (fw >> 8) & 0xfffu);
        return pcc::invalid(buf);
    }
    const bool split_enabled = pcc::tuning(PCC_TUNE_AM_NOSPLIT) == 0;

    struct Lane {
        int s0, bc;
        hipStream_t st;
        WsView v;
        Sched sc;
    };
    Lane lanes[kMaxLanes];
    int nlanes = 1;
    bool fork = false;
    if (split_enabled && L.b >= 8 && (long long)L.b * std::max(L.n, L.m) >= 32768) {
        fork = !pcc::capturing(st);
    }
    ForkJoin fj(st, fork);
    if (fj.side) nlanes = 2;
    for (int l = 0; l < nlanes; l++) {
        Lane &ln = lanes[l];
        ln.s0 = (int)((long long)L.b * l / nlanes);
        ln.bc = (int)((long long)L.b * (l + 1) / nlanes) - ln.s0;
        ln.st = l == 0 ? st : fj.side;
        ln.v = L.view(base, ln.s0);
        ln.sc = lane_sched(L, ln.v, lc);
    }
    int rc = PCC_OK;
    auto enqueue_head = [&](int l) -> int {
        const Lane &ln = lanes[l];
        const size_t s0 = (size_t)ln.s0;
        int r = pcc::sort_clouds(L, ln.v, ln.bc, xyz1 + s0 * L.n * 3, xyz2 + s0 * L.m * 3, (bool)after_sort, ln.st);
        if (!r && after_sort && l % 2 == 0) r = after_sort(ln.s0, ln.bc, ln.st);
        return r;
    };
    auto enqueue_pass = [&](int l, int p) -> int {
        const Lane &ln = lanes[l];
        int mode, var;
        const PhaseArgs a = build_phase(ln.sc, p, &mode, &var);
        switch (mode) {
        case PH_A: return launch_phase<PH_A>(a, ln.bc, var, ln.st, "approxmatch(A)");
        case PH_B: return launch_phase<PH_B>(a, ln.bc, var, ln.st, "approxmatch(B)");
        case PH_CA: return launch_phase<PH_CA>(a, ln.bc, var, ln.st, "approxmatch(CA)");
        default: return launch_phase<PH_C>(a, ln.bc, var, ln.st, "approxmatch(C)");
        }
    };
    int first_pass[kMaxLanes] = {};
    {
        for (int l = 0; l < nlanes && !rc; l++) rc = enqueue_head(l);
        if (rc) return rc;
        {
            pcc::ProfScope seq0("am_phase_sequence", lanes[0].st, true);
            pcc::ProfScope seq1("am_phase_sequence", lanes[nlanes > 1 ? 1 : 0].st, true, nlanes >= 2);
            for (int l = 0; l < nlanes && !rc; l++) {
                const int r = launch_fine_resident(lanes[l].sc, lanes[l].bc, lanes[l].st);
                if (r > 0) rc = r;
                else if (r == 0) first_pass[l] = kFpPasses;
            }
            for (int p = 0; p < sched_phases() && !rc; p++)
                for (int l = 0; l < nlanes && !rc; l++)
                    if (p >= first_pass[l]) rc = enqueue_pass(l, p);
            if (rc) return rc;
        }
        if (after_sort)
            for (int l = 1; l < nlanes; l += 2)
                if (int rc2 = after_sort(lanes[l].s0, lanes[l].bc, lanes[l].st)) return rc2;
        if (lane_tail) {
            for (int l = 0; l < nlanes; l++)
                if (int rc2 = lane_tail(lanes[l].s0, lanes[l].bc, lanes[l].st)) return rc2;
        }
    }
    return PCC_OK;
}

int approxmatch_impl(int b, int n, int m, const float *xyz1, const float *xyz2, float *match, float *temp,
                     void *workspace, size_t workspace_bytes, float *cost_out, hipStream_t st) {
    const WsLayout L(b, n, m);
    if (workspace_bytes < L.total) return pcc::invalid("approxmatch: workspace too small");
    if (!aligned16(workspace)) return pcc::invalid("approxmatch: workspace must be 16-byte aligned");
    char *base = static_cast<char *>(workspace);
    const LevelConsts lc = make_levels();
    int rc = run_levels(L, base, xyz1, xyz2, lc, st);
    if (rc) return rc;
    const WsView v = L.view(base, 0);
    hipLaunchKernelGGL(am_unpermute_kernel, dim3(pcc::ceil_div(n + m, 256), b), dim3(256), 0, st, n, m, L.n4, L.m4, v.lv, v.rem,
                       v.rank1, v.rank2, v.live_cnt, v.lv_orig, temp);
    rc = pcc::check_launch("approxmatch(unpermute)");
    if (rc) return rc;
    const dim3 grid(pcc::ceil_div(n, kMatKT), pcc::ceil_div(m, kMatLT), b);
    const bool vec = (n % 4 == 0) && aligned16(match);
    if (cost_out) {
        {
            pcc::ProfScope prof("am_materialise_kernel<cost>", st);
            if (vec) hipLaunchKernelGGL((am_materialise_kernel<true, true>), grid, dim3(256), 0, st, n, m, xyz1, xyz2, v.lv_orig, lc, match, v.cpart);
            else hipLaunchKernelGGL((am_materialise_kernel<true, false>), grid, dim3(256), 0, st, n, m, xyz1, xyz2, v.lv_orig, lc, match, v.cpart);
        }
        rc = pcc::check_launch("approxmatch(materialise+cost)");
        if (rc) return rc;
        pcc::launch_reduce_rows(b, (int)cost_parts(n, m), v.cpart, cost_out, st);
        return pcc::check_launch("approxmatch(cost reduce)");
    }
    {
        pcc::ProfScope prof("am_materialise_kernel", st);
        if (vec) hipLaunchKernelGGL((am_materialise_kernel<false, true>), grid, dim3(256), 0, st, n, m, xyz1, xyz2, v.lv_orig, lc, match, nullptr);
        else hipLaunchKernelGGL((am_materialise_kernel<false, false>), grid, dim3(256), 0, st, n, m, xyz1, xyz2, v.lv_orig, lc, match, nullptr);
    }
    return pcc::check_launch("approxmatch(materialise)");
}

int match_cost_implicit_impl(int b, int n, int m, const float *xyz1, const float *xyz2, const float *grad_cost,
                             float *cost, float *grad1, float *grad2, hipStream_t st,
                             const pcc::ChamferOut *chamfer = nullptr) {
    const bool grad = grad1 && grad2;
    const int col_blocks = pcc::ceil_div(n, 64 * kPairQ), row_tiles = pcc::ceil_div(m, kPairRT);
    const WsLayout L(b, n, m, col_blocks, row_tiles, grad);
    pcc::WsBlock ws(st);
    if (int rc = ws.alloc(L.total, "workspace allocation failed")) return rc;
    char *base = static_cast<char *>(ws.p);
    const LevelConsts lc = make_levels();
    auto tail = [&](int s0, int bc, hipStream_t lst) -> int {
        return pcc::launch_pair_finish(L, L.view(base, s0), s0, bc, col_blocks, row_tiles, grad_cost, cost, grad1, grad2, chamfer, lst);
    };
    auto nn_after_sort = [&](int s0, int bc, hipStream_t lst) -> int {
        return pcc::launch_nn_sorted(L, L.view(base, s0), s0, bc, chamfer, lst);
    };
    if (chamfer) return run_levels(L, base, xyz1, xyz2, lc, st, tail, nn_after_sort);
    return run_levels(L, base, xyz1, xyz2, lc, st, tail);
}

int approxmatch_entry(int b, int n, int m, const float *xyz1, const float *xyz2, float *match, float *temp, bool with_cost,
                      float *cost, hipStream_t st) {
    pcc::clear_error();
    if (int rc = check_sizes(with_cost ? "approxmatch_cost" : "approxmatch", b, n, m)) return rc;
    const char *null_ptr = with_cost ? "approxmatch_cost: null pointer" : "approxmatch: null pointer";
    if (b == 0) return PCC_OK;
    if (with_cost && !cost) return pcc::invalid(null_ptr);
    if (n == 0 || m == 0)
        return with_cost ? zero_fill_empty(b, n, m, cost, nullptr, nullptr, st, "approxmatch_cost: memset failed") : PCC_OK;
    if (!xyz1 || !xyz2 || !match || !temp) return pcc::invalid(null_ptr);
    pcc::WsBlock ws(st);
    const size_t bytes = WsLayout(b, n, m).total;
    if (int rc = ws.alloc(bytes, "workspace allocation failed")) return rc;
    return approxmatch_impl(b, n, m, xyz1, xyz2, match, temp, ws.p, bytes, cost, st);
}

}

namespace pcc {
int match_cost_with_chamfer(int b, int n, int m, const float *xyz1, const float *xyz2, float *cost, float *grad1,
                            float *grad2, hipStream_t st, const ChamferOut &chamfer) {
    return match_cost_implicit_impl(b, n, m, xyz1, xyz2, nullptr, cost, grad1, grad2, st, &chamfer);
}

}

extern "C" {

size_t pcc_approxmatch_workspace_bytes(int b, int n, int m) {
    if (b <= 0 || n <= 0 || m <= 0) return 0;
    return WsLayout(b, n, m).total;
}

int pcc_approxmatch_ws(int b, int n, int m, const float *xyz1, const float *xyz2, float *match, float *temp,
                       void *workspace, size_t workspace_bytes, pcc_stream_t stream) {
    pcc::clear_error();
    if (int rc = check_sizes("approxmatch", b, n, m)) return rc;
    if (b == 0 || n == 0 || m == 0) return PCC_OK;
    if (!xyz1 || !xyz2 || !match || !temp || !workspace) return pcc::invalid("approxmatch: null pointer");
    return approxmatch_impl(b, n, m, xyz1, xyz2, match, temp, workspace, workspace_bytes, nullptr,
                            static_cast<hipStream_t>(stream));
}

int pcc_approxmatch(int b, int n, int m, const float *xyz1, const float *xyz2, float *match, float *temp,
                    pcc_stream_t stream) {
    return approxmatch_entry(b, n, m, xyz1, xyz2, match, temp, false, nullptr, static_cast<hipStream_t>(stream));
}

int pcc_approxmatch_cost(int b, int n, int m, const float *xyz1, const float *xyz2, float *match, float *temp,
                         float *cost, pcc_stream_t stream) {
    return approxmatch_entry(b, n, m, xyz1, xyz2, match, temp, true, cost, static_cast<hipStream_t>(stream));
}

int pcc_match_cost(int b, int n, int m, const float *xyz1, const float *xyz2, const float *grad_cost, float *cost,
                   float *grad1, float *grad2, pcc_stream_t stream) {
    pcc::clear_error();
    if (int rc = check_sizes("match_cost", b, n, m)) return rc;
    if (b == 0) return PCC_OK;
    if (!cost) return pcc::invalid("match_cost: null pointer");
    hipStream_t st = static_cast<hipStream_t>(stream);
    if (n == 0 || m == 0) return zero_fill_empty(b, n, m, cost, grad1, grad2, st, "match_cost: memset failed");
    if (!xyz1 || !xyz2) return pcc::invalid("match_cost: null pointer");
    if ((grad1 == nullptr) != (grad2 == nullptr)) return pcc::invalid("match_cost: grad1 and grad2 go together");
    return match_cost_implicit_impl(b, n, m, xyz1, xyz2, grad_cost, cost, grad1, grad2, st);
}

void approxmatch(int b, int n, int m, const float *xyz1, const float *xyz2, float *match, float *temp,
                 pcc_stream_t stream) {
    (void)pcc_approxmatch(b, n, m, xyz1, xyz2, match, temp, stream);
}

}
```

pointcloudcounterfactual_amd/csrc/approxmatch.hpp:

```cpp
#pragma once
#include "pcc_common.hpp"

namespace {

using pcc::v4f;

constexpr int kLevels = 9;
constexpr float kLog2e = 1.44269504088896340736f;

struct LevelConsts {
    float c[kLevels];
};

inline LevelConsts make_levels() {
    LevelConsts lc;
    float level = -16384.0f;
    for (int i = 0; i < kLevels; i++) {
        lc.c[i] = level * kLog2e;
        level *= 0.25f;
    }
    return lc;
}

__device__ __forceinline__ float fast_exp2(float x) { return __builtin_amdgcn_exp2f(x); }

using pcc::kBox;
constexpr int kLiveRow = 16;
constexpr int kInfSlot = 13;
constexpr float kZeroExp = 151.f;
constexpr int kBarSlot = 12;
constexpr int kErrSlot = 15;
constexpr int kPairRT = 128;
constexpr int kPairQ = 4;

inline int mask_words(int m4) { return (m4 + 31) / 32; }

inline float zero_cut2(const LevelConsts &lc, int i) { return kZeroExp / -lc.c[i]; }

inline bool aligned16(const void *p) { return (reinterpret_cast<uintptr_t>(p) & 15) == 0; }

inline int check_sizes(const char *who, int b, int n, int m) {
    if (b < 0 || n < 0 || m < 0) return pcc::invalidf("%s: bad size", who);
    if ((long long)n * 3 > 0x7fffffffLL || (long long)m * 3 > 0x7fffffffLL) return pcc::invalidf("%s: bad size", who);
    if (b > 65535) return pcc::invalidf("%s: batch too large", who);
    return PCC_OK;
}

inline int zero_fill_empty(int b, int n, int m, float *cost, float *grad1, float *grad2, hipStream_t st, const char *what) {
    int rc = PCC_OK;
    if (cost) rc = pcc::zero_async(cost, (size_t)b * sizeof(float), st, what);
    if (n && grad1 && !rc) rc = pcc::zero_async(grad1, (size_t)b * n * 3 * sizeof(float), st, what);
    if (m && grad2 && !rc) rc = pcc::zero_async(grad2, (size_t)b * m * 3 * sizeof(float), st, what);
    return rc;
}

}

namespace pcc {

struct AmDims {
    int n, m, n4, m4, nb1, nb2;
    AmDims(int n_, int m_) : n(n_), m(m_), n4((n_ + 3) & ~3), m4((m_ + 3) & ~3), nb1(ceil_div(n_, kBox)), nb2(ceil_div(m_, kBox)) {}
    size_t rem_floats() const { return (size_t)n4 + 2 * (size_t)m4; }
    size_t lv_floats() const { return kLevels * ((size_t)n4 + m4); }
};

struct WsView {
    float *soa1, *soa2;
    int *rank1, *rank2, *perm1, *perm2;
    float *box1, *box2;
    float *rem;
    float *lv;
    float *lv_orig;
    float *cpart;
    float *clist;
    int *clist_cnt;
    int *live_cnt;
    unsigned *live_mask;
    float4 *aos1, *aos2;
    float *pair_cost, *part1, *part2;
};

int sort_clouds(const AmDims &L, const WsView &v, int bc, const float *xyz1, const float *xyz2, bool aos, hipStream_t st);
int launch_nn_sorted(const AmDims &L, const WsView &v, int s0, int bc, const ChamferOut *chamfer, hipStream_t lst);
int launch_pair_finish(const AmDims &L, const WsView &v, int s0, int bc, int col_blocks, int row_tiles, const float *grad_cost,
                       float *cost, float *grad1, float *grad2, const ChamferOut *chamfer, hipStream_t lst);
void launch_reduce_rows(int b, int parts, const float *part, float *out, hipStream_t st);

}
```

pointcloudcounterfactual_amd/csrc/chamfer.hip:

```cpp
#include "pcc_common.hpp"

namespace {

using pcc::kWave;
using pcc::sq3;

constexpr int kGroup = 8;

template <int R, int S, int CH>
__global__ __launch_bounds__(64 * S) void nn_fwd_kernel(int b, int n, const float *__restrict__ xyz, int m,
                                                         const float *__restrict__ xyz2,
                                                         float *__restrict__ res1, int *__restrict__ idx1,
                                                         float *__restrict__ res2, int *__restrict__ idx2,
                                                         int tiles_n, int tiles_m) {
    constexpr int T = 64 * S;
    constexpr int TQ = 64 * R;
    static_assert(CH % (kGroup * 4) == 0, "chunk must hold whole float4 groups");
    __shared__ __attribute__((aligned(16))) float lds_c[3 * CH];
    __shared__ float red_best[S][TQ];
    __shared__ int red_idx[S][TQ];
    __shared__ float run_best[TQ];
    __shared__ int run_idx[TQ];

    const int tid = threadIdx.x;
    const int lane = tid & 63;
    const int w = __builtin_amdgcn_readfirstlane(tid >> 6);

    int bid = pcc::xcd_contiguous((int)blockIdx.x, (int)gridDim.x);
    const int dir0 = b * tiles_n;
    const float *Q, *C;
    float *out_d;
    int *out_i;
    int nq, nc, tiles;
    if (bid < dir0) {
        Q = xyz; C = xyz2; nq = n; nc = m; tiles = tiles_n; out_d = res1; out_i = idx1;
    } else {
        bid -= dir0;
        Q = xyz2; C = xyz; nq = m; nc = n; tiles = tiles_m; out_d = res2; out_i = idx2;
    }
    const int smp = bid / tiles;
    const int tile = bid - smp * tiles;
    Q += (size_t)smp * nq * 3;
    C += (size_t)smp * nc * 3;
    out_d += (size_t)smp * nq;
    out_i += (size_t)smp * nq;

    float qx[R], qy[R], qz[R];
#pragma unroll
    for (int r = 0; r < R; r++) {
        int q = tile * TQ + r * 64 + lane;
        q = q < nq ? q : nq - 1;
        qx[r] = Q[q * 3 + 0];
        qy[r] = Q[q * 3 + 1];
        qz[r] = Q[q * 3 + 2];
    }
    for (int e = tid; e < TQ; e += T) {
        run_best[e] = __builtin_inff();
        run_idx[e] = 0;
    }

    const float4 *X4 = reinterpret_cast<const float4 *>(lds_c);
    const float4 *Y4 = X4 + CH / 4;
    const float4 *Z4 = Y4 + CH / 4;

    for (int c0 = 0; c0 < nc; c0 += CH) {
        const int cnt = min(CH, nc - c0);
        const int ngroups = (cnt + kGroup - 1) / kGroup;
        __syncthreads();
        const float *src = C + (size_t)c0 * 3;
        for (int i = tid; i < cnt * 3; i += T) {
            float v = src[i];
            int p = i / 3;
            int c = i - p * 3;
            lds_c[c * CH + p] = v;
        }
        for (int i = cnt + tid; i < ngroups * kGroup; i += T) {
            lds_c[i] = __builtin_inff();
            lds_c[CH + i] = __builtin_inff();
            lds_c[2 * CH + i] = __builtin_inff();
        }
        __syncthreads();

        const int gs = (ngroups + S - 1) / S;
        const int g_begin = w * gs;
        const int g_end = min(g_begin + gs, ngroups);

        float cb[R];
        int cg[R];
#pragma unroll
        for (int r = 0; r < R; r++) {
            cb[r] = __builtin_inff();
            cg[r] = min(g_begin, ngroups - 1);
        }
        for (int g = g_begin; g < g_end; g++) {
            const float4 xa = X4[2 * g], xb = X4[2 * g + 1];
            const float4 ya = Y4[2 * g], yb = Y4[2 * g + 1];
            const float4 za = Z4[2 * g], zb = Z4[2 * g + 1];
#pragma unroll
            for (int r = 0; r < R; r++) {
                const float d0 = sq3(xa.x - qx[r], ya.x - qy[r], za.x - qz[r]);
                const float d1 = sq3(xa.y - qx[r], ya.y - qy[r], za.y - qz[r]);
                const float d2 = sq3(xa.z - qx[r], ya.z - qy[r], za.z - qz[r]);
                const float d3 = sq3(xa.w - qx[r], ya.w - qy[r], za.w - qz[r]);
                const float d4 = sq3(xb.x - qx[r], yb.x - qy[r], zb.x - qz[r]);
                const float d5 = sq3(xb.y - qx[r], yb.y - qy[r], zb.y - qz[r]);
                const float d6 = sq3(xb.z - qx[r], yb.z - qy[r], zb.z - qz[r]);
                const float d7 = sq3(xb.w - qx[r], yb.w - qy[r], zb.w - qz[r]);
                float mn = __builtin_fminf(__builtin_fminf(d0, d1), d2);
                mn = __builtin_fminf(__builtin_fminf(mn, d3), d4);
                mn = __builtin_fminf(__builtin_fminf(mn, d5), d6);
                mn = __builtin_fminf(mn, d7);
                const bool lt = mn < cb[r];
                cb[r] = lt ? mn : cb[r];
                cg[r] = lt ? g : cg[r];
            }
        }
#pragma unroll
        for (int r = 0; r < R; r++) {
            const int base = cg[r] * kGroup;
            int found = 0;
#pragma unroll
            for (int c = kGroup - 1; c >= 0; c--) {
                const float d = sq3(lds_c[base + c] - qx[r], lds_c[CH + base + c] - qy[r],
                                    lds_c[2 * CH + base + c] - qz[r]);
                found = (d == cb[r]) ? c : found;
            }
            red_best[w][r * 64 + lane] = cb[r];
            red_idx[w][r * 64 + lane] = c0 + base + found;
        }
        __syncthreads();
        for (int e = tid; e < TQ; e += T) {
            float rb = run_best[e];
            int ri = run_idx[e];
#pragma unroll
            for (int s = 0; s < S; s++) {
                const float v = red_best[s][e];
                const bool lt = v < rb;
                ri = lt ? red_idx[s][e] : ri;
                rb = lt ? v : rb;
            }
            run_best[e] = rb;
            run_idx[e] = ri;
        }
    }
    __syncthreads();
    for (int e = tid; e < TQ; e += T) {
        const int q = tile * TQ + e;
        if (q < nq) {
            float rb = run_best[e];
            int ri = run_idx[e];
            const float ux = Q[q * 3 + 0], uy = Q[q * 3 + 1], uz = Q[q * 3 + 2];
            const float d0 = sq3(C[0] - ux, C[1] - uy, C[2] - uz);
            if (d0 != d0 || !(rb < __builtin_inff())) {
                rb = d0;
                ri = 0;
            }
            bool quirk = false;
            for (int h = 512; h < nc; h += 512) {
                const float dh = sq3(C[h * 3 + 0] - ux, C[h * 3 + 1] - uy, C[h * 3 + 2] - uz);
                quirk |= (dh != dh);
            }
            if (quirk && d0 == d0) {
                for (int k2 = 0; k2 < nc; k2 += 512) {
                    const int end_k = min(nc, k2 + 512);
                    float best = 0.f;
                    int best_i = 0;
                    for (int k = k2; k < end_k; k++) {
                        const float d = sq3(C[k * 3 + 0] - ux, C[k * 3 + 1] - uy, C[k * 3 + 2] - uz);
                        if (k == k2 || d < best) {
                            best = d;
                            best_i = k;
                        }
                    }
                    if (k2 == 0 || rb > best) {
                        rb = best;
                        ri = best_i;
                    }
                }
            }
            out_d[q] = rb;
            out_i[q] = ri;
        }
    }
}

__global__ __launch_bounds__(256) void nn_bwd_range_kernel(int n, const float *__restrict__ xyz1, int m,
                                                            const float *__restrict__ xyz2,
                                                            const float *__restrict__ gd1,
                                                            const int *__restrict__ idx1,
                                                            const float *__restrict__ gd2,
                                                            const int *__restrict__ idx2,
                                                            float *__restrict__ grad1, float *__restrict__ grad2,
                                                            int P, const float *__restrict__ gloss, int mean, int gloss_stride,
                                                            const float *__restrict__ add1,
                                                            const float *__restrict__ add2,
                                                            const float *__restrict__ add_scale, int add_stride) {
    extern __shared__ __attribute__((aligned(16))) float acc[];
    const int lid = pcc::xcd_contiguous((int)blockIdx.x, (int)gridDim.x);
    const int smp = lid / P, p = lid - smp * P;
    const int tid = threadIdx.x, T = 256;
    const int j0 = (int)((long long)n * p / P), j1 = (int)((long long)n * (p + 1) / P);
    const int k0 = (int)((long long)m * p / P), k1 = (int)((long long)m * (p + 1) / P);
    float *acc1 = acc;
    float *acc2 = acc + (j1 - j0) * 3;
    const float *p1 = xyz1 + (size_t)smp * n * 3;
    const float *p2 = xyz2 + (size_t)smp * m * 3;
    const int *i1 = idx1 + (size_t)smp * n;
    const int *i2 = idx2 + (size_t)smp * m;
    const float *g1 = gloss ? nullptr : gd1 + (size_t)smp * n;
    const float *g2 = gloss ? nullptr : gd2 + (size_t)smp * m;
    const float gs = gloss ? gloss[(size_t)smp * gloss_stride] : 0.f;
    const float gs1 = mean ? gs / (float)n : gs, gs2 = mean ? gs / (float)m : gs;
    for (int j = j0 + tid; j < j1; j += T) {
        const int j2 = i1[j];
        const float g = (gloss ? gs1 : g1[j]) * 2;
#pragma unroll
        for (int c = 0; c < 3; c++) acc1[(j - j0) * 3 + c] = g * (p1[j * 3 + c] - p2[j2 * 3 + c]);
    }
    for (int k = k0 + tid; k < k1; k += T) {
        const int k2 = i2[k];
        const float g = (gloss ? gs2 : g2[k]) * 2;
#pragma unroll
        for (int c = 0; c < 3; c++) acc2[(k - k0) * 3 + c] = g * (p2[k * 3 + c] - p1[k2 * 3 + c]);
    }
    __syncthreads();
    for (int k = tid; k < m; k += T) {
        const int j = i2[k];
        if (j >= j0 && j < j1) {
            const float g = (gloss ? gs2 : g2[k]) * 2;
#pragma unroll
            for (int c = 0; c < 3; c++) atomicAdd(&acc1[(j - j0) * 3 + c], -(g * (p2[k * 3 + c] - p1[j * 3 + c])));
        }
    }
    for (int j = tid; j < n; j += T) {
        const int k = i1[j];
        if (k >= k0 && k < k1) {
            const float g = (gloss ? gs1 : g1[j]) * 2;
#pragma unroll
            for (int c = 0; c < 3; c++) atomicAdd(&acc2[(k - k0) * 3 + c], -(g * (p1[j * 3 + c] - p2[k * 3 + c])));
        }
    }
    __syncthreads();
    float *o1 = grad1 + ((size_t)smp * n + j0) * 3;
    float *o2 = grad2 + ((size_t)smp * m + k0) * 3;
    if (add1) {
        const float as = add_scale ? add_scale[(size_t)smp * add_stride] : 1.0f;
        const float *a1 = add1 + ((size_t)smp * n + j0) * 3;
        const float *a2 = add2 + ((size_t)smp * m + k0) * 3;
        for (int i = tid; i < (j1 - j0) * 3; i += T) o1[i] = acc1[i] + a1[i] * as;
        for (int i = tid; i < (k1 - k0) * 3; i += T) o2[i] = acc2[i] + a2[i] * as;
        return;
    }
    for (int i = tid; i < (j1 - j0) * 3; i += T) o1[i] = acc1[i];
    for (int i = tid; i < (k1 - k0) * 3; i += T) o2[i] = acc2[i];
}

__global__ __launch_bounds__(256) void chamfer_reduce_kernel(int n, int m, const float *__restrict__ dist1,
                                                              const float *__restrict__ dist2, int mean,
                                                              float *__restrict__ loss) {
    __shared__ float red[2][256];
    const int smp = blockIdx.x, tid = threadIdx.x;
    float s1 = 0.f, s2 = 0.f;
    for (int i = tid; i < n; i += 256) s1 += dist1[(size_t)smp * n + i];
    for (int i = tid; i < m; i += 256) s2 += dist2[(size_t)smp * m + i];
    red[0][tid] = s1;
    red[1][tid] = s2;
    __syncthreads();
    for (int off = 128; off > 0; off >>= 1) {
        if (tid < off) {
            red[0][tid] += red[0][tid + off];
            red[1][tid] += red[1][tid + off];
        }
        __syncthreads();
    }
    if (tid == 0) loss[smp] = mean ? red[1][0] / (float)m + red[0][0] / (float)n : red[0][0] + red[1][0];
}

int launch_bwd(int b, int n, const float *xyz1, int m, const float *xyz2, const float *grad_dist1, const int *idx1,
               const float *grad_dist2, const int *idx2, const float *gloss, int mean, int gloss_stride,
               float *grad_xyz1, float *grad_xyz2, hipStream_t st, const float *add1 = nullptr,
               const float *add2 = nullptr, const float *add_scale = nullptr, int add_stride = 1) {
    long long P = std::max<long long>(1, pcc::ceil_div(512, b));
    P = std::min<long long>(P, std::max(1, std::min(n, m) / 64));
    const long long lds_min = ((long long)n + m) * 12 / (48 * 1024) + 1;
    P = std::max(P, lds_min);
    if (P * b > 0x7fffffffLL) return pcc::invalid("nndistancegrad: clouds too large");
    const size_t lds = ((size_t)pcc::ceil_div(n, (int)P) + pcc::ceil_div(m, (int)P) + 2) * 3 * sizeof(float);
    {
        pcc::ProfScope prof("nn_bwd_range_kernel", st);
        hipLaunchKernelGGL(nn_bwd_range_kernel, dim3((unsigned)(P * b)), dim3(256), lds, st, n, xyz1, m, xyz2,
                           grad_dist1, idx1, grad_dist2, idx2, grad_xyz1, grad_xyz2, (int)P, gloss, mean, gloss_stride,
                           add1, add2, add_scale, add_stride);
    }
    return pcc::check_launch("nndistancegrad");
}

template <int R, int S>
int launch_fwd(int b, int n, const float *xyz, int m, const float *xyz2, float *res1, int *idx1, float *res2,
               int *idx2, hipStream_t st) {
    constexpr int CH = 2048;
    const int tiles_n = pcc::ceil_div(n, 64 * R), tiles_m = pcc::ceil_div(m, 64 * R);
    const long long grid = (long long)b * (tiles_n + tiles_m);
    if (grid > 0x7fffffffLL) return pcc::invalid("nndistance: grid too large");
    {
        pcc::ProfScope prof("nn_fwd_kernel", st);
        hipLaunchKernelGGL((nn_fwd_kernel<R, S, CH>), dim3((unsigned)grid), dim3(64 * S), 0, st, b, n, xyz, m, xyz2,
                           res1, idx1, res2, idx2, tiles_n, tiles_m);
    }
    return pcc::check_launch("nndistance");
}

}

extern "C" {

int pcc_nndistance(int b, int n, const float *xyz, int m, const float *xyz2, float *result, int *result_i,
                   float *result2, int *result2_i, pcc_stream_t stream) {
    pcc::clear_error();
    if (b < 0 || n < 0 || m < 0) return pcc::invalid("nndistance: negative size");
    if (b == 0 || (n == 0 && m == 0)) return PCC_OK;
    if (n == 0 || m == 0) return pcc::invalid("nndistance: one cloud is empty (reference leaves outputs undefined)");
    if (!xyz || !xyz2 || !result || !result_i || !result2 || !result2_i) return pcc::invalid("nndistance: null pointer");
    hipStream_t st = static_cast<hipStream_t>(stream);
    const long long queries = (long long)b * ((long long)n + m);
    if (queries >= 256LL * 64 * 8) return launch_fwd<4, 4>(b, n, xyz, m, xyz2, result, result_i, result2, result2_i, st);
    if (queries >= 256LL * 64 * 2) return launch_fwd<2, 4>(b, n, xyz, m, xyz2, result, result_i, result2, result2_i, st);
    return launch_fwd<1, 4>(b, n, xyz, m, xyz2, result, result_i, result2, result2_i, st);
}

void nndistance(int b, int n, const float *xyz, int m, const float *xyz2, float *result, int *result_i,
                float *result2, int *result2_i, pcc_stream_t stream) {
    (void)pcc_nndistance(b, n, xyz, m, xyz2, result, result_i, result2, result2_i, stream);
}

int pcc_nndistancegrad(int b, int n, const float *xyz1, int m, const float *xyz2, const float *grad_dist1,
                       const int *idx1, const float *grad_dist2, const int *idx2, float *grad_xyz1,
                       float *grad_xyz2, pcc_stream_t stream) {
    pcc::clear_error();
    if (b < 0 || n < 0 || m < 0) return pcc::invalid("nndistancegrad: negative size");
    if (b == 0 || (n == 0 && m == 0)) return PCC_OK;
    if (n == 0 || m == 0) return pcc::invalid("nndistancegrad: one cloud is empty");
    if (!xyz1 || !xyz2 || !grad_dist1 || !idx1 || !grad_dist2 || !idx2 || !grad_xyz1 || !grad_xyz2)
        return pcc::invalid("nndistancegrad: null pointer");
    return launch_bwd(b, n, xyz1, m, xyz2, grad_dist1, idx1, grad_dist2, idx2, nullptr, 0, 1, grad_xyz1, grad_xyz2,
                      static_cast<hipStream_t>(stream));
}

int pcc_chamfer_loss(int b, int n, const float *xyz1, int m, const float *xyz2, int mean, float *loss, float *dist1,
                     int *idx1, float *dist2, int *idx2, pcc_stream_t stream) {
    if (int rc = pcc_nndistance(b, n, xyz1, m, xyz2, dist1, idx1, dist2, idx2, stream)) return rc;
    if (b == 0) return PCC_OK;
    if (!loss) return pcc::invalid("chamfer_loss: null pointer");
    hipStream_t st = static_cast<hipStream_t>(stream);
    hipLaunchKernelGGL(chamfer_reduce_kernel, dim3((unsigned)b), dim3(256), 0, st, n, m, dist1, dist2, mean, loss);
    return pcc::check_launch("chamfer_loss(reduce)");
}

int pcc_chamfer_loss_grad(int b, int n, const float *xyz1, int m, const float *xyz2, const int *idx1, const int *idx2,
                          const float *grad_loss, int grad_loss_stride, int mean, float *grad_xyz1, float *grad_xyz2,
                          pcc_stream_t stream) {
    pcc::clear_error();
    if (b < 0 || n < 0 || m < 0) return pcc::invalid("chamfer_loss_grad: negative size");
    if (b == 0 || (n == 0 && m == 0)) return PCC_OK;
    if (n == 0 || m == 0) return pcc::invalid("chamfer_loss_grad: one cloud is empty");
    if (!xyz1 || !xyz2 || !idx1 || !idx2 || !grad_loss || !grad_xyz1 || !grad_xyz2)
        return pcc::invalid("chamfer_loss_grad: null pointer");
    if (grad_loss_stride != 0 && grad_loss_stride != 1) return pcc::invalid("chamfer_loss_grad: grad_loss stride must be 0 or 1");
    return launch_bwd(b, n, xyz1, m, xyz2, nullptr, idx1, nullptr, idx2, grad_loss, mean, grad_loss_stride, grad_xyz1, grad_xyz2,
                      static_cast<hipStream_t>(stream));
}

int pcc_chamfer_emd(int b, int n, const float *xyz1, int m, const float *xyz2, int mean, float *chamfer_loss,
                    float *dist1, int *idx1, float *dist2, int *idx2, float *emd_cost, float *emd_grad1,
                    float *emd_grad2, pcc_stream_t stream) {
    pcc::clear_error();
    if (b < 0 || n < 0 || m < 0) return pcc::invalid("chamfer_emd: negative size");
    if (b == 0) return PCC_OK;
    if (n == 0 || m == 0) return pcc::invalid("chamfer_emd: one cloud is empty");
    if ((long long)n * 3 > 0x7fffffffLL || (long long)m * 3 > 0x7fffffffLL) return pcc::invalid("chamfer_emd: bad size");
    if (b > 65535) return pcc::invalid("chamfer_emd: batch too large");
    if (!xyz1 || !xyz2 || !chamfer_loss || !dist1 || !idx1 || !dist2 || !idx2 || !emd_cost)
        return pcc::invalid("chamfer_emd: null pointer");
    if ((emd_grad1 == nullptr) != (emd_grad2 == nullptr)) return pcc::invalid("chamfer_emd: emd_grad1 and emd_grad2 go together");
    const pcc::ChamferOut ch{mean, chamfer_loss, dist1, dist2, idx1, idx2};
    return pcc::match_cost_with_chamfer(b, n, m, xyz1, xyz2, emd_cost, emd_grad1, emd_grad2,
                                        static_cast<hipStream_t>(stream), ch);
}

int pcc_chamfer_emd_grad(int b, int n, const float *xyz1, int m, const float *xyz2, const int *idx1, const int *idx2,
                         const float *grad_chamfer, int grad_chamfer_stride, int mean, const float *emd_grad1,
                         const float *emd_grad2, const float *grad_emd, int grad_emd_stride, float *grad_xyz1,
                         float *grad_xyz2, pcc_stream_t stream) {
    pcc::clear_error();
    if (b < 0 || n < 0 || m < 0) return pcc::invalid("chamfer_emd_grad: negative size");
    if (b == 0 || (n == 0 && m == 0)) return PCC_OK;
    if (n == 0 || m == 0) return pcc::invalid("chamfer_emd_grad: one cloud is empty");
    if (!xyz1 || !xyz2 || !idx1 || !idx2 || !grad_chamfer || !emd_grad1 || !emd_grad2 || !grad_xyz1 || !grad_xyz2)
        return pcc::invalid("chamfer_emd_grad: null pointer");
    if ((grad_chamfer_stride != 0 && grad_chamfer_stride != 1) || (grad_emd_stride != 0 && grad_emd_stride != 1))
        return pcc::invalid("chamfer_emd_grad: gradient strides must be 0 or 1");
    return launch_bwd(b, n, xyz1, m, xyz2, nullptr, idx1, nullptr, idx2, grad_chamfer, mean, grad_chamfer_stride, grad_xyz1,
                      grad_xyz2, static_cast<hipStream_t>(stream), emd_grad1, emd_grad2, grad_emd, grad_emd_stride);
}

void nndistancegrad(int b, int n, const float *xyz1, int m, const float *xyz2, const float *grad_dist1,
                    const int *idx1, const float *grad_dist2, const int *idx2, float *grad_xyz1, float *grad_xyz2,
                    pcc_stream_t stream) {
    (void)pcc_nndistancegrad(b, n, xyz1, m, xyz2, grad_dist1, idx1, grad_dist2, idx2, grad_xyz1, grad_xyz2, stream);
}

}
```

pointcloudcounterfactual_amd/losses.py:

```python

from __future__ import annotations

import math
from typing import Any

import torch
from torch.autograd import Function

from pointcloudcounterfactual_amd import backend


class NNDistanceFunction(Function):

    @staticmethod
    def forward(ctx: Any, *args: Any, **kwargs: Any) -> Any:
        set1, set2, *_ = args
        ctx.save_for_backward(set1, set2)
        dist1, idx1, dist2, idx2 = backend.NNDistance(set1, set2)
        ctx.idx1 = idx1
        ctx.idx2 = idx2
        return dist1, dist2

    @staticmethod
    def backward(ctx: Any, *grad_outputs: Any) -> Any:
        set1, set2 = ctx.saved_tensors
        grad1, grad2 = backend.NNDistanceGrad(
            set1, set2, ctx.idx1, ctx.idx2, grad_outputs[0].contiguous(), grad_outputs[1].contiguous()
        )
        return grad1, grad2


class MatchCostFunction(Function):

    mode = 'implicit'

    @staticmethod
    def forward(ctx: Any, *args: torch.Tensor, **kwargs: Any) -> torch.Tensor:
        set1, set2, *_ = args
        mode = MatchCostFunction.mode
        ctx.mode = mode
        if mode == 'implicit':
            with_grad = bool(ctx.needs_input_grad[0] or ctx.needs_input_grad[1])
            out = backend.MatchCostImplicit(set1, set2, with_grad)
            if with_grad:
                ctx.save_for_backward(out[1], out[2])
            return out[0]
        ctx.save_for_backward(set1, set2)
        if mode == 'fused':
            match, _temp, cost = backend.ApproxMatchCost(set1, set2)
        elif mode == 'reference':
            match, _temp = backend.ApproxMatch(set1, set2)
            cost = backend.MatchCost(set1, set2, match)
        else:
            raise ValueError(f'unknown MatchCostFunction.mode {mode!r}')
        ctx.match = match
        return cost

    @staticmethod
    def backward(ctx: Any, *grad_outputs: Any) -> tuple[torch.Tensor, torch.Tensor]:
        grad_output = grad_outputs[0]
        if ctx.mode == 'implicit':
            grad1, grad2 = ctx.saved_tensors
            scale = grad_output.unsqueeze(1).unsqueeze(2)
            return (grad1 * scale if ctx.needs_input_grad[0] else None,
                    grad2 * scale if ctx.needs_input_grad[1] else None)
        set1, set2 = ctx.saved_tensors
        if ctx.mode == 'fused':
            grad1, grad2 = backend.MatchCostGradScaled(set1, set2, ctx.match, grad_output.contiguous().float())
            return grad1, grad2
        grad1, grad2 = backend.MatchCostGrad(set1, set2, ctx.match)
        scale = grad_output.unsqueeze(1).unsqueeze(2)
        return grad1 * scale, grad2 * scale

    @classmethod
    def apply(cls, x: torch.Tensor, y: torch.Tensor) -> torch.Tensor:
        return super().apply(x, y)


nn_distance = NNDistanceFunction.apply
match_cost = MatchCostFunction.apply


class ChamferFunction(Function):

    @staticmethod
    def forward(ctx: Any, *args: Any, **kwargs: Any) -> torch.Tensor:
        t1, t2, mean = args
        loss, _d1, idx1, _d2, idx2 = backend.ChamferLoss(t1, t2, bool(mean))
        ctx.save_for_backward(t1, t2, idx1, idx2)
        ctx.mean = bool(mean)
        return loss

    @staticmethod
    def backward(ctx: Any, *grad_outputs: Any) -> Any:
        t1, t2, idx1, idx2 = ctx.saved_tensors
        g = grad_outputs[0]
        grad1, grad2 = backend.ChamferLossGrad(t1, t2, idx1, idx2, g if g.dtype == torch.float32 else g.float(), ctx.mean)
        return grad1, grad2, None


def chamfer(t1: torch.Tensor, t2: torch.Tensor, reduction: str = 'mean') -> torch.Tensor:
    if reduction not in ('mean', 'sum'):
        raise ValueError(f"reduction must be 'mean' or 'sum', got {reduction!r}")
    return ChamferFunction.apply(t1, t2, reduction == 'mean')


class ChamferEMDFunction(Function):

    @staticmethod
    def forward(ctx: Any, *args: Any, **kwargs: Any) -> Any:
        t1, t2, mean = args
        with_grad = bool(ctx.needs_input_grad[0] or ctx.needs_input_grad[1])
        out = backend.ChamferEMD(t1, t2, bool(mean), with_grad)
        if with_grad:
            ctx.save_for_backward(t1, t2, out[1], out[2], out[4], out[5])
        ctx.mean = bool(mean)
        return out[0], out[3]

    @staticmethod
    def backward(ctx: Any, *grad_outputs: Any) -> Any:
        t1, t2, idx1, idx2, e1, e2 = ctx.saved_tensors
        gc, ge = grad_outputs
        gc = gc if gc.dtype == torch.float32 else gc.float()
        ge = ge if ge.dtype == torch.float32 else ge.float()
        grad1, grad2 = backend.ChamferEMDGrad(t1, t2, idx1, idx2, gc, ctx.mean, e1, e2, ge)
        return (grad1 if ctx.needs_input_grad[0] else None, grad2 if ctx.needs_input_grad[1] else None, None)


def chamfer_emd(t1: torch.Tensor, t2: torch.Tensor, reduction: str = 'mean') -> tuple[torch.Tensor, torch.Tensor]:
    if reduction not in ('mean', 'sum'):
        raise ValueError(f"reduction must be 'mean' or 'sum', got {reduction!r}")
    return ChamferEMDFunction.apply(t1, t2, reduction == 'mean')


def torch_square_distance(t1: torch.Tensor, t2: torch.Tensor) -> torch.Tensor:
    t2 = t2.transpose(-1, -2)
    dist = -2 * torch.matmul(t1, t2)
    dist += torch.sum(t1**2, -1, keepdim=True)
    dist += torch.sum(t2**2, -2, keepdim=True)
    return dist


def torch_chamfer(t1: torch.Tensor, t2: torch.Tensor) -> torch.Tensor:
    dist = torch_square_distance(t1, t2)
    return torch.min(dist, dim=-1)[0].sum(1) + torch.min(dist, dim=-2)[0].sum(1)


def random_directions(p: int, device: torch.device | str, generator: torch.Generator | None = None) -> torch.Tensor:
    device = torch.device(device)
    raw = torch.randn(p, 3, generator=generator, device=device if generator is None else generator.device)
    return torch.nn.functional.normalize(raw, dim=1).to(device)


def _sw_forward(t1: torch.Tensor, t2: torch.Tensor, theta: torch.Tensor) -> tuple[torch.Tensor, ...]:
    n, p = t1.size(1), theta.size(0)

    def sorted_projection(t: torch.Tensor) -> tuple[torch.Tensor, torch.Tensor]:
        v, th = t[:, None, :, :], theta[None, :, None, :]
        proj = (v[..., 0] * th[..., 0] + v[..., 1] * th[..., 1]) + v[..., 2] * th[..., 2]
        proj = torch.where(proj == 0, torch.zeros_like(proj), proj)
        return torch.sort(proj, dim=2, stable=True)

    (a, perm1), (b, perm2) = sorted_projection(t1), sorted_projection(t2)
    d = a - b
    size = 1 << max(n - 1, 0).bit_length()
    e = torch.zeros(d.shape[:2] + (size,), dtype=d.dtype)
    e[..., :n] = d * d
    while size > 1:
        size //= 2
        e = e[..., :size] + e[..., size:2 * size]
    cost_p = e[..., 0]
    total = cost_p[:, 0]
    for k in range(1, p):
        total = total + cost_p[:, k]
    inv = torch.tensor(1.0 / (float(n) * float(p)), dtype=torch.float64).to(torch.float32)
    return total * inv, cost_p, d, perm1, perm2, inv


class TorchSlicedWassersteinFunction(Function):

    @staticmethod
    def forward(ctx: Any, *args: Any, **kwargs: Any) -> torch.Tensor:
        t1, t2, theta = args
        cost, _cost_p, d, perm1, perm2, inv = _sw_forward(t1, t2, theta)
        ctx.save_for_backward(d, perm1, perm2, theta, inv)
        return cost

    @staticmethod
    def backward(ctx: Any, *grad_outputs: Any) -> Any:
        d, perm1, perm2, theta, inv = ctx.saved_tensors
        g = grad_outputs[0]
        scale = ((g if g.dtype == torch.float32 else g.float()) * (2 * inv))[:, None, None]

        def grad(perm: torch.Tensor, diff: torch.Tensor) -> torch.Tensor:
            by_point = torch.empty_like(diff).scatter_(2, perm, diff)
            return torch.einsum('bpn,pc->bnc', by_point, theta) * scale

        return (grad(perm1, d) if ctx.needs_input_grad[0] else None, grad(perm2, -d) if ctx.needs_input_grad[1] else None, None)


def torch_sliced_wasserstein(t1: torch.Tensor, t2: torch.Tensor, directions: torch.Tensor,
                             return_per_direction: bool = False) -> Any:
    for name, t in (('t1', t1), ('t2', t2), ('directions', directions)):
        if t.dtype != torch.float32:
            raise RuntimeError(f'{name} must be torch.float32, found {t.dtype}')
    if t1.dim() != 3 or t1.size(2) != 3 or t2.shape != t1.shape or t1.size(1) < 1:
        raise ValueError(f'clouds must be [B,N,3] of one shape with N >= 1, got {tuple(t1.shape)} and {tuple(t2.shape)}')
    if directions.dim() != 2 or directions.size(1) != 3 or directions.size(0) < 1:
        raise ValueError(f'directions must be [P,3] with P >= 1, got {tuple(directions.shape)}')
    cost = TorchSlicedWassersteinFunction.apply(t1, t2, directions)
    if return_per_direction:
        with torch.no_grad():
            return cost, _sw_forward(t1, t2, directions)[1]
    return cost


class SlicedWassersteinFunction(Function):

    @staticmethod
    def forward(ctx: Any, *args: Any, **kwargs: Any) -> torch.Tensor:
        t1, t2, theta = args
        need1, need2 = bool(ctx.needs_input_grad[0]), bool(ctx.needs_input_grad[1])
        cost, _cost_p, g1, g2 = backend.SlicedWasserstein(t1, t2, theta, need1, need2)
        ctx.save_for_backward(*(g for g in (g1, g2) if g is not None))
        ctx.needs = (need1, need2)
        return cost

    @staticmethod
    def backward(ctx: Any, *grad_outputs: Any) -> Any:
        saved = list(ctx.saved_tensors)
        g = grad_outputs[0]
        scale = (g if g.dtype == torch.float32 else g.float())[:, None, None]
        grad1 = saved.pop(0) * scale if ctx.needs[0] else None
        grad2 = saved.pop(0) * scale if ctx.needs[1] else None
        return grad1, grad2, None


def sliced_wasserstein(t1: torch.Tensor, t2: torch.Tensor, n_projections: int = 128, directions: torch.Tensor | None = None,
                       generator: torch.Generator | None = None) -> torch.Tensor:
    if directions is None:
        directions = random_directions(n_projections, t1.device, generator)
    if t1.device.type == 'cpu':
        return torch_sliced_wasserstein(t1, t2, directions)
    return SlicedWassersteinFunction.apply(t1, t2, directions)


def sinkhorn_schedule(blur: float, scaling: float, diameter: float) -> list[float]:
    if not (blur > 0 and diameter > 0 and 0 < scaling < 1) or not all(math.isfinite(v) for v in (blur, scaling, diameter)):
        raise ValueError(f'sinkhorn_schedule: need blur > 0, diameter > 0 and 0 < scaling < 1, got {blur}, {scaling}, {diameter}')
    start, stop, step = 2 * math.log(diameter), 2 * math.log(blur), 2 * math.log(scaling)
    count = max(0, math.ceil((stop - start) / step))
    return [diameter**2] + [math.exp(start + i * step) for i in range(count)] + [blur**2]


def _halving_tree(e: torch.Tensor) -> torch.Tensor:
    n = e.size(-1)
    size = 1 << max(n - 1, 0).bit_length()
    pad = torch.zeros(e.shape[:-1] + (size,), dtype=e.dtype, device=e.device)
    pad[..., :n] = e
    while size > 1:
        size //= 2
        pad = pad[..., :size] + pad[..., size:2 * size]
    return pad[..., 0]


def _sk_forward(t1: torch.Tensor, t2: torch.Tensor, eps: list[float], debias: bool) -> tuple[torch.Tensor, ...]:
    n, m = t1.size(1), t2.size(1)

    def pairs(u: torch.Tensor, v: torch.Tensor) -> tuple[torch.Tensor, torch.Tensor]:
        diff = u[:, :, None, :] - v[:, None, :, :]
        return diff, 0.5 * (diff * diff).sum(-1)

    def softmin(e: float, cost: torch.Tensor, h: torch.Tensor | None) -> torch.Tensor:
        arg = -cost / e if h is None else (h[:, None, :] - cost) / e
        return -e * torch.logsumexp(arg - math.log(cost.size(2)), dim=2)

    (dxy, cxy), (dyx, cyx) = pairs(t1, t2), pairs(t2, t1)
    f, g = softmin(eps[0], cxy, None), softmin(eps[0], cyx, None)
    if debias:
        dxx, cxx = pairs(t1, t1)
        dyy, cyy = pairs(t2, t2)
        p, q = softmin(eps[0], cxx, None), softmin(eps[0], cyy, None)
    for e in eps:
        f, g = 0.5 * (f + softmin(e, cxy, g)), 0.5 * (g + softmin(e, cyx, f))
        if debias:
            p, q = 0.5 * (p + softmin(e, cxx, p)), 0.5 * (q + softmin(e, cyy, q))
    e = eps[-1]

    def plan_grad(cost: torch.Tensor, diff: torch.Tensor, h: torch.Tensor) -> torch.Tensor:
        return torch.einsum('bij,bijc->bic', torch.softmax((h[:, None, :] - cost) / e, dim=2), diff)

    pot1, pot2 = softmin(e, cxy, g), softmin(e, cyx, f)
    grad1, grad2 = plan_grad(cxy, dxy, g), plan_grad(cyx, dyx, f)
    if debias:
        pot1, pot2 = pot1 - softmin(e, cxx, p), pot2 - softmin(e, cyy, q)
        grad1, grad2 = grad1 - plan_grad(cxx, dxx, p), grad2 - plan_grad(cyy, dyy, q)
    inv_n = torch.tensor(1.0 / n, dtype=torch.float64).to(torch.float32)
    inv_m = torch.tensor(1.0 / m, dtype=torch.float64).to(torch.float32)
    cost = inv_n * _halving_tree(pot1) + inv_m * _halving_tree(pot2)
    return cost, pot1, pot2, inv_n * grad1, inv_m * grad2


def _sk_check(t1: torch.Tensor, t2: torch.Tensor, eps: list[float] | None) -> None:
    for name, t in (('t1', t1), ('t2', t2)):
        if t.dtype != torch.float32:
            raise RuntimeError(f'{name} must be torch.float32, found {t.dtype}')
    if t1.dim() != 3 or t2.dim() != 3 or t1.size(2) != 3 or t2.size(2) != 3 or t1.size(0) != t2.size(0) or t1.size(1) < 1 or t2.size(1) < 1:
        raise ValueError(f'clouds must be [B,N,3] and [B,M,3] with N, M >= 1, got {tuple(t1.shape)} and {tuple(t2.shape)}')
    if eps is not None and (not 1 <= len(eps) <= 256 or not all(math.isfinite(e) and e > 0 for e in eps)):
        raise ValueError('eps must hold 1 to 256 finite temperatures > 0')


class _SinkhornBase(Function):

    @staticmethod
    def run(t1: torch.Tensor, t2: torch.Tensor, eps: list[float], debias: bool, need1: bool, need2: bool, potentials: bool) -> Any:
        raise NotImplementedError

    @classmethod
    def forward(cls, ctx: Any, *args: Any, **kwargs: Any) -> Any:
        t1, t2, eps, debias, potentials, grad_mode = args
        need1, need2 = bool(grad_mode and ctx.needs_input_grad[0]), bool(grad_mode and ctx.needs_input_grad[1])
        cost, p1, p2, g1, g2 = cls.run(t1, t2, eps, debias, need1, need2, potentials)
        ctx.save_for_backward(*(g for g in (g1, g2) if g is not None))
        ctx.needs = (need1, need2)
        if potentials:
            ctx.mark_non_differentiable(p1, p2)
        return cost, p1, p2

    @staticmethod
    def backward(ctx: Any, *grad_outputs: Any) -> Any:
        saved = list(ctx.saved_tensors)
        g = grad_outputs[0]
        scale = (g if g.dtype == torch.float32 else g.float())[:, None, None]
        grad1 = saved.pop(0) * scale if ctx.needs[0] else None
        grad2 = saved.pop(0) * scale if ctx.needs[1] else None
        return grad1, grad2, None, None, None, None


class TorchSinkhornFunction(_SinkhornBase):

    @staticmethod
    def run(t1: torch.Tensor, t2: torch.Tensor, eps: list[float], debias: bool, need1: bool, need2: bool, potentials: bool) -> Any:
        cost, p1, p2, g1, g2 = _sk_forward(t1, t2, eps, debias)
        return cost, p1 if potentials else None, p2 if potentials else None, g1 if need1 else None, g2 if need2 else None


class SinkhornFunction(_SinkhornBase):

    @staticmethod
    def run(t1: torch.Tensor, t2: torch.Tensor, eps: list[float], debias: bool, need1: bool, need2: bool, potentials: bool) -> Any:
        return backend.Sinkhorn(t1, t2, eps, debias, need1, need2, potentials)


def torch_sinkhorn(t1: torch.Tensor, t2: torch.Tensor, eps: list[float], debias: bool = True, return_potentials: bool = False) -> Any:
    eps = [float(e) for e in eps]
    _sk_check(t1, t2, eps)
    cost, p1, p2 = TorchSinkhornFunction.apply(t1, t2, eps, bool(debias), bool(return_potentials), torch.is_grad_enabled())
    return (cost, p1, p2) if return_potentials else cost


def sinkhorn_divergence(t1: torch.Tensor, t2: torch.Tensor, blur: float = 0.05, scaling: float = 0.5, diameter: float | None = None,
                        eps: list[float] | None = None, debias: bool = True, return_potentials: bool = False) -> Any:
    _sk_check(t1, t2, None)
    if eps is None:
        if diameter is None:
            both = torch.cat((t1.detach().reshape(-1, t1.size(-1)), t2.detach().reshape(-1, t2.size(-1))))
            diameter = float((both.max(0).values.double() - both.min(0).values.double()).max())
            if not diameter > 0:
                diameter = float(blur)
        eps = sinkhorn_schedule(float(blur), float(scaling), float(diameter))
    eps = [float(e) for e in eps]
    _sk_check(t1, t2, eps)
    fn = TorchSinkhornFunction if t1.device.type == 'cpu' else SinkhornFunction
    cost, p1, p2 = fn.apply(t1, t2, eps, bool(debias), bool(return_potentials), torch.is_grad_enabled())
    return (cost, p1, p2) if return_potentials else cost
```

Baseline: 73130 clouds/s.

## Fuse first-cloud EMD gradient accumulation into approxmatch pass C when only grad1 needed

Adds a path for the case where only the first cloud needs a gradient. In that case the per-point cost and gradient sums are accumulated inside the approxmatch pass-C and fine kernels, and the separate pair kernel is skipped. It also plumbs a grad2 flag through the Python autograd functions so the second gradient is not allocated or computed. This removes a full pair pass, at the cost of extra per-candidate work (rsqrt plus FMAs) and register and LDS pressure in the pass-C kernels. It also disables the resident fine path when this mode is active.

```diff
diff --git a/pointcloudcounterfactual_amd/backend.py b/pointcloudcounterfactual_amd/backend.py
--- a/pointcloudcounterfactual_amd/backend.py
+++ b/pointcloudcounterfactual_amd/backend.py
@@ -38,7 +38,7 @@
     return [match, temp, cost]
 
 
-def MatchCostImplicit(set_d: torch.Tensor, set_q: torch.Tensor, with_grad: bool) -> list[torch.Tensor]:
+def MatchCostImplicit(set_d: torch.Tensor, set_q: torch.Tensor, with_grad: bool, grad2: bool = True) -> list[torch.Tensor | None]:
     b, n, m = _sizes(set_d, set_q)
     dev = set_d.device
     cost = torch.empty((b,), dtype=torch.float32, device=dev)
@@ -46,7 +46,7 @@
     g1 = g2 = None
     if with_grad:
         g1 = torch.empty((b, n, 3), dtype=torch.float32, device=dev)
-        g2 = torch.empty((b, m, 3), dtype=torch.float32, device=dev)
+        g2 = torch.empty((b, m, 3), dtype=torch.float32, device=dev) if grad2 else None
         out += [g1, g2]
     call(_L.pcc_match_cost, 'MatchCostImplicit', dev, b, n, m, ptr(set_d, 'set_d', F32, dev),
          ptr(set_q, 'set_q', F32, dev), None, ptr(cost, 'cost', F32, dev), ptr(g1, 'grad1', F32, dev),
@@ -136,7 +136,7 @@
 
 
 def ChamferEMD(set_d: torch.Tensor, set_q: torch.Tensor, mean: bool, with_grad: bool,
-               return_dist: bool = False) -> list[torch.Tensor]:
+               return_dist: bool = False, grad2: bool = True) -> list[torch.Tensor | None]:
     b, n, m = _sizes(set_d, set_q)
     dev = set_d.device
     loss = torch.empty((b,), dtype=torch.float32, device=dev)
@@ -147,7 +147,7 @@
     g1 = g2 = None
     if with_grad:
         g1 = torch.empty((b, n, 3), dtype=torch.float32, device=dev)
-        g2 = torch.empty((b, m, 3), dtype=torch.float32, device=dev)
+        g2 = torch.empty((b, m, 3), dtype=torch.float32, device=dev) if grad2 else None
         out += [g1, g2]
     d1 = torch.empty((b, n), dtype=torch.float32, device=dev)
     d2 = torch.empty((b, m), dtype=torch.float32, device=dev)
@@ -170,23 +170,23 @@
 
 
 def ChamferEMDGrad(set_d: torch.Tensor, set_q: torch.Tensor, idx1: torch.Tensor, idx2: torch.Tensor,
-                   grad_chamfer: torch.Tensor, mean: bool, emd_grad1: torch.Tensor, emd_grad2: torch.Tensor,
-                   grad_emd: torch.Tensor) -> list[torch.Tensor]:
+                   grad_chamfer: torch.Tensor, mean: bool, emd_grad1: torch.Tensor, emd_grad2: torch.Tensor | None,
+                   grad_emd: torch.Tensor) -> list[torch.Tensor | None]:
     b, n, m = _sizes(set_d, set_q)
     dev = set_d.device
     grad1 = torch.empty((b, n, 3), dtype=torch.float32, device=dev)
     grad2 = torch.empty((b, m, 3), dtype=torch.float32, device=dev)
     if (idx1.numel() != b * n or idx2.numel() != b * m or grad_chamfer.numel() != b or grad_emd.numel() != b
-            or emd_grad1.numel() != b * n * 3 or emd_grad2.numel() != b * m * 3):
+            or emd_grad1.numel() != b * n * 3 or (emd_grad2 is not None and emd_grad2.numel() != b * m * 3)):
         raise RuntimeError('ChamferEMDGrad: shapes do not match the clouds')
     grad_chamfer, sc = _batch_stride(grad_chamfer, b)
     grad_emd, se = _batch_stride(grad_emd, b)
     call(_L.pcc_chamfer_emd_grad, 'ChamferEMDGrad', dev, b, n, ptr(set_d, 'set_d', F32, dev), m,
          ptr(set_q, 'set_q', F32, dev), ptr(idx1, 'idx1', I32, dev), ptr(idx2, 'idx2', I32, dev),
          ptr(grad_chamfer, 'grad_chamfer', F32, dev), sc, int(mean), ptr(emd_grad1, 'emd_grad1', F32, dev),
-         ptr(emd_grad2, 'emd_grad2', F32, dev), ptr(grad_emd, 'grad_emd', F32, dev), se, ptr(grad1, 'grad1', F32, dev),
-         ptr(grad2, 'grad2', F32, dev))
-    return [grad1, grad2]
+         ptr(set_q if emd_grad2 is None else emd_grad2, 'emd_grad2', F32, dev), ptr(grad_emd, 'grad_emd', F32, dev), se,
+         ptr(grad1, 'grad1', F32, dev), ptr(grad2, 'grad2', F32, dev))
+    return [grad1, None if emd_grad2 is None else grad2]
 
 
 def NNDistanceGrad(set_d: torch.Tensor, set_q: torch.Tensor, idx1: torch.Tensor, idx2: torch.Tensor,
diff --git a/pointcloudcounterfactual_amd/csrc/am_pair.hip b/pointcloudcounterfactual_amd/csrc/am_pair.hip
--- a/pointcloudcounterfactual_amd/csrc/am_pair.hip
+++ b/pointcloudcounterfactual_amd/csrc/am_pair.hip
@@ -310,6 +310,7 @@
     const size_t o = (size_t)s0;
     const int n = L.n, m = L.m;
     const bool grad = grad1 && grad2;
+    const bool first = grad1 && !grad2;
     const LevelConsts lc = make_levels();
     PairArgs pa{};
     pa.n = n; pa.m = m; pa.n4 = L.n4; pa.m4 = L.m4;
@@ -322,14 +323,19 @@
     pa.col_blocks = col_blocks; pa.row_tiles = row_tiles; pa.bc = bc;
     if ((long long)col_blocks * row_tiles * bc > 0x7fffffffLL) return pcc::invalid("match_cost: grid too large");
     const dim3 grid((unsigned)(col_blocks * row_tiles * bc));
-    if (int rc = launch_pair<kPairQ>(pa, grid, grad, lst)) return rc;
+    if (!first)
+        if (int rc = launch_pair<kPairQ>(pa, grid, grad, lst)) return rc;
     FinishArgs f{};
     f.parts[0] = row_tiles; f.parts[1] = col_blocks; f.parts[2] = col_blocks * row_tiles;
     f.npts[0] = n; f.npts[1] = m; f.pitch[0] = L.n4; f.pitch[1] = L.m4;
     f.part[0] = pa.part1; f.part[1] = pa.part2; f.part[2] = pa.cost_part;
+    if (first) {
+        f.parts[0] = 1; f.parts[2] = n;
+        f.part[0] = v.fg_grad; f.part[2] = v.fg_cost;
+    }
     f.perm[0] = v.perm1; f.perm[1] = v.perm2;
     f.scale = grad_cost ? grad_cost + o : nullptr;
-    f.out[0] = grad ? grad1 + o * n * 3 : nullptr;
+    f.out[0] = grad1 ? grad1 + o * n * 3 : nullptr;
     f.out[1] = grad ? grad2 + o * m * 3 : nullptr;
     f.out[2] = cost + o;
     f.flags = v.live_cnt;
@@ -339,7 +345,7 @@
     }
     {
         pcc::ProfScope prof("pair_finish_kernel", lst);
-        const int blocks = grad ? pcc::ceil_div(std::max(n, m) * 3, 256) : 1;
+        const int blocks = grad ? pcc::ceil_div(std::max(n, m) * 3, 256) : first ? pcc::ceil_div(n * 3, 256) : 1;
         hipLaunchKernelGGL(pair_finish_kernel, dim3(blocks, bc, chamfer ? 4 : 3), dim3(256), 0, lst, f);
     }
     return pcc::check_launch("match_cost(reduce)");
diff --git a/pointcloudcounterfactual_amd/csrc/approxmatch.hip b/pointcloudcounterfactual_amd/csrc/approxmatch.hip
--- a/pointcloudcounterfactual_amd/csrc/approxmatch.hip
+++ b/pointcloudcounterfactual_amd/csrc/approxmatch.hip
@@ -24,6 +24,38 @@
     return {consumption * remR, __builtin_fmaxf(0.0f, remR - sumr)};
 }
 __device__ __forceinline__ float pass_c_left(float remL, float ratioL, float sum) { return __builtin_fmaxf(0.0f, remL - ratioL * sum); }
+
+struct FgSums {
+    float c, x, y, z;
+};
+__device__ __forceinline__ void fg_add(FgSums &s, float e, float wa, float d, float dx, float dy, float dz) {
+    float dm;
+    asm("v_max_f32 %0, %1, %2" : "=v"(dm) : "v"(d), "v"(1e-20f));
+    const float f = (e * wa) * __builtin_amdgcn_rsqf(dm);
+    s.c = __builtin_fmaf(f, d, s.c);
+    s.x = __builtin_fmaf(dx, f, s.x);
+    s.y = __builtin_fmaf(dy, f, s.y);
+    s.z = __builtin_fmaf(dz, f, s.z);
+}
+struct FgOld {
+    float c, x, y, z;
+};
+__device__ __forceinline__ FgOld fg_fetch(const float *grad_row, const float *cost_row, int o, bool first) {
+    FgOld v = {0.f, 0.f, 0.f, 0.f};
+    if (!first) {
+        v.c = cost_row[o];
+        v.x = grad_row[(size_t)o * 3];
+        v.y = grad_row[(size_t)o * 3 + 1];
+        v.z = grad_row[(size_t)o * 3 + 2];
+    }
+    return v;
+}
+__device__ __forceinline__ void fg_store(float *grad_row, float *cost_row, int o, const FgOld &old, float ratioL, const FgSums &t) {
+    cost_row[o] = __builtin_fmaf(ratioL, t.c, old.c);
+    grad_row[(size_t)o * 3] = __builtin_fmaf(ratioL, -t.x, old.x);
+    grad_row[(size_t)o * 3 + 1] = __builtin_fmaf(ratioL, -t.y, old.y);
+    grad_row[(size_t)o * 3 + 2] = __builtin_fmaf(ratioL, -t.z, old.z);
+}
 
 struct PhaseArgs {
     int n_own, n_cand, tiles, batch;
@@ -54,6 +86,7 @@
     int mask_words;
     const int *live_in;
     int *live_out;
+    float *fg_grad, *fg_cost;
 };
 
 enum Var { V_PLAIN = 0, V_CULL = 1, V_COWN = 3, V_CLIST = 4 };
@@ -68,6 +101,7 @@
     int *live_cnt;
     unsigned *live_mask;
     int skip;
+    float *fg_grad, *fg_cost;
     LevelConsts lc;
 };
 
@@ -134,6 +168,7 @@
             a.w1 = sc.rem + sc.n4 + ((i + 1) & 1) * sc.m4; a.w1_stride = rs;
             a.remain = sc.rem; a.remain_stride = rs;
             a.ratio_in = ratioL; a.ratio_stride = kLevels * nm4;
+            a.fg_grad = sc.fg_grad; a.fg_cost = sc.fg_cost;
             const int lc_i = i + 1 < kLevels ? i + 1 : i;
             a.cut2 = zero_cut2(sc.lc, lc_i);
             a.cut2_fine = zero_cut2(sc.lc, i);
@@ -148,16 +183,19 @@
     return a;
 }
 
-template <int NW, int R, int S, int CH>
+template <int NW, int R, int S, int CH, bool FG = false>
 struct PhaseLds {
     static constexpr int kC = (3 + NW) * CH;
     static constexpr int kRed = NW * S * 64 * R;
     static constexpr int kOwn = 64 * R;
     static constexpr int kWave = S;
-    static constexpr int floats = kC + kRed + kOwn + kWave + 4;
+    static constexpr int kBase = kC + kRed + kOwn + kWave + 4;
+    static constexpr int kFg = FG ? 4 * S * 64 * R : 0;
+    static constexpr bool kFgInC = kFg <= kC;
+    static constexpr int floats = kBase + (kFgInC ? 0 : kFg);
 };
 
-template <int MODE, int R, int S, int CH, int VAR, int G = 1>
+template <int MODE, int R, int S, int CH, int VAR, int G = 1, bool FG = false>
 __device__ __forceinline__ void am_phase_body(const PhaseArgs &a, int smp, int tile, float *smem) {
     constexpr int T = 64 * S;
     constexpr int TQ = 64 * R / G;
@@ -169,7 +207,8 @@
     static_assert(VAR == V_PLAIN || COWN || CLIST, "the box-culled passes run on am_fine_kernel");
     static_assert(!(CLIST && W0_CONST), "pass A of the first level has constant weights");
     static_assert(TQ <= T, "one epilogue owner per thread");
-    using L = PhaseLds<NW, R, S, CH>;
+    static_assert(!FG || ((MODE == PH_CA || MODE == PH_C) && G == 1), "first-cloud sums: pass C only");
+    using L = PhaseLds<NW, R, S, CH, FG>;
     float *lds_c = smem;
     float *red = smem + L::kC;
     int *own_idx = reinterpret_cast<int *>(red + L::kRed);
@@ -274,6 +313,16 @@
         const int oe = max(own_e, 0);
         if (MODE != PH_A && !a.first) pre_rem = a.remain[(size_t)smp * a.remain_stride + oe];
         if (MODE == PH_CA || MODE == PH_C) pre_ratio = a.ratio_in[(size_t)smp * a.ratio_stride + oe];
+    }
+    float *fg_grow = nullptr, *fg_crow = nullptr;
+    FgOld fg_old = {0.f, 0.f, 0.f, 0.f};
+    FgSums fg[R], fg_odd = {0.f, 0.f, 0.f, 0.f};
+    if (FG) {
+        fg_grow = a.fg_grad + (size_t)smp * 3 * a.own_n4;
+        fg_crow = a.fg_cost + (size_t)smp * a.n_own;
+        fg_old = fg_fetch(fg_grow, fg_crow, max(own_e, 0), a.first);
+#pragma unroll
+        for (int r = 0; r < R; r++) fg[r] = {0.f, 0.f, 0.f, 0.f};
     }
     const float4 *X4 = reinterpret_cast<const float4 *>(lds_c);
     const float4 *Y4 = X4 + CH / 4;
@@ -331,6 +380,30 @@
                 const float4 x = X4[g], y = Y4[g], z = Z4[g], wa = A4[g];
                 float4 wb;
                 if (NW == 2) wb = B4[g];
+                if (FG) {
+#pragma unroll
+                    for (int r = 0; r < R; r++) {
+                        const float cx[4] = {x.x, x.y, x.z, x.w}, cy[4] = {y.x, y.y, y.z, y.w}, cz[4] = {z.x, z.y, z.z, z.w};
+                        const float va[4] = {wa.x, wa.y, wa.z, wa.w};
+                        float vb[4] = {0.f, 0.f, 0.f, 0.f};
+                        if (NW == 2) { vb[0] = wb.x; vb[1] = wb.y; vb[2] = wb.z; vb[3] = wb.w; }
+#pragma unroll
+                        for (int q = 0; q < 4; q++) {
+                            const float dx = cx[q] - ox[r], dy = cy[q] - oy[r], dz = cz[q] - oz[r];
+                            const float d = sq3(dx, dy, dz);
+                            const float e = fast_exp2(c0 * d);
+                            const bool odd = R == 1 && (q & 1);
+                            if (odd) t0x = __builtin_fmaf(e, va[q], t0x);
+                            else s0[r] = __builtin_fmaf(e, va[q], s0[r]);
+                            fg_add(odd ? fg_odd : fg[r], e, va[q], d, dx, dy, dz);
+                            if (NW == 2) {
+                                if (odd) t1x = __builtin_fmaf(fast_exp2(c1 * d), vb[q], t1x);
+                                else s1[r] = __builtin_fmaf(fast_exp2(c1 * d), vb[q], s1[r]);
+                            }
+                        }
+                    }
+                    continue;
+                }
 #pragma unroll
                 for (int r = 0; r < R; r++) {
                     const float d0 = sq3(x.x - ox[r], y.x - oy[r], z.x - oz[r]);
@@ -377,8 +450,34 @@
         red[(0 * S + w) * PQ + r * 64 + lane] = s0[r];
         if (NW == 2) red[(1 * S + w) * PQ + r * 64 + lane] = s1[r];
     }
+    float *fg_red = L::kFgInC ? lds_c : smem + L::kBase;
+    if (FG) {
+        if (R == 1) {
+            fg[0].c += fg_odd.c; fg[0].x += fg_odd.x; fg[0].y += fg_odd.y; fg[0].z += fg_odd.z;
+        }
+        __syncthreads();
+#pragma unroll
+        for (int r = 0; r < R; r++) {
+            fg_red[(0 * S + w) * PQ + r * 64 + lane] = fg[r].c;
+            fg_red[(1 * S + w) * PQ + r * 64 + lane] = fg[r].x;
+            fg_red[(2 * S + w) * PQ + r * 64 + lane] = fg[r].y;
+            fg_red[(3 * S + w) * PQ + r * 64 + lane] = fg[r].z;
+        }
+    }
     __syncthreads();
     if (own_e < 0) return;
+    if (FG) {
+        const int e = tid;
+        FgSums t = {fg_red[e], fg_red[(1 * S) * PQ + e], fg_red[(2 * S) * PQ + e], fg_red[(3 * S) * PQ + e]};
+#pragma unroll
+        for (int s = 1; s < S; s++) {
+            t.c += fg_red[(0 * S + s) * PQ + e];
+            t.x += fg_red[(1 * S + s) * PQ + e];
+            t.y += fg_red[(2 * S + s) * PQ + e];
+            t.z += fg_red[(3 * S + s) * PQ + e];
+        }
+        fg_store(fg_grow, fg_crow, own_e, fg_old, pre_ratio, t);
+    }
     {
         const int e = tid;
         const int o = own_e;
@@ -425,9 +524,9 @@
     }
 }
 
-template <int MODE, int R, int S, int CH, int VAR, int G = 1>
-__global__ __launch_bounds__(64 * S) void am_phase_kernel(PhaseArgs a) {
-    __shared__ __attribute__((aligned(16))) float smem[PhaseLds<(MODE == PH_CA ? 2 : 1), R, S, CH>::floats];
+template <int MODE, int R, int S, int CH, int VAR, int G = 1, bool FG = false>
+__global__ __launch_bounds__(64 * S, (FG && R == 1 && MODE == PH_CA) ? 8 : 2) void am_phase_kernel(PhaseArgs a) {
+    __shared__ __attribute__((aligned(16))) float smem[PhaseLds<(MODE == PH_CA ? 2 : 1), R, S, CH, FG>::floats];
     constexpr bool COWN = VAR == V_COWN;
     int smp, tile;
     const int bid = (int)blockIdx.x, nwg = (int)gridDim.x;
@@ -446,7 +545,7 @@
         smp = lid / a.tiles;
         tile = lid - smp * a.tiles;
     }
-    am_phase_body<MODE, R, S, CH, VAR, G>(a, smp, tile, smem);
+    am_phase_body<MODE, R, S, CH, VAR, G, FG>(a, smp, tile, smem);
 }
 
 constexpr int kFineS = 8;
@@ -495,9 +594,10 @@
     __syncthreads();
 }
 
-template <int NW>
+template <int NW, bool FG = false>
 __device__ __forceinline__ void fine_walk(const FineRows &rows, const unsigned char *list, int nitems, int cs, int cl, float c0,
-                                          float c1, const FineOwners &own, float (&s0)[kFineQ], float (&s1)[kFineQ]) {
+                                          float c1, const FineOwners &own, float (&s0)[kFineQ], float (&s1)[kFineQ],
+                                          FgSums *fg = nullptr) {
     for (int it = cs; it < nitems; it += 2) {
         const int item = __builtin_amdgcn_readfirstlane((int)list[it]);
         const int ci = (item & 127) * kBox + cl;
@@ -513,40 +613,57 @@
         if (NW == 2) wb = rows.w1[ci];
 #pragma unroll
         for (int j = 0; j < kFineQ; j++) {
-            const float d = sq3(x - own.x[j], y - own.y[j], z - own.z[j]);
-            s0[j] = __builtin_fmaf(fast_exp2(c0 * d), wa, s0[j]);
+            const float dx = x - own.x[j], dy = y - own.y[j], dz = z - own.z[j];
+            const float d = sq3(dx, dy, dz);
+            const float e = fast_exp2(c0 * d);
+            s0[j] = __builtin_fmaf(e, wa, s0[j]);
+            if (FG) fg_add(fg[j], e, wa, d, dx, dy, dz);
             if (NW == 2) s1[j] = __builtin_fmaf(fast_exp2(c1 * d), wb, s1[j]);
         }
     }
 }
 
-template <int NW>
-__device__ __forceinline__ void fine_reduce(float (&s0)[kFineQ], float (&s1)[kFineQ], float (*red)[2][64], int cs, int cl, int og, int quad) {
+template <int NW, bool FG = false>
+__device__ __forceinline__ void fine_reduce(float (&s0)[kFineQ], float (&s1)[kFineQ], float (*red)[2][64], int cs, int cl, int og, int quad,
+                                            FgSums *fg = nullptr) {
     const auto add = [](float a, float b) { return a + b; };
 #pragma unroll
     for (int j = 0; j < kFineQ; j++) {
         s0[j] = pcc::row_reduce16(s0[j], add);
         if (NW == 2) s1[j] = pcc::row_reduce16(s1[j], add);
+        if (FG) {
+            fg[j].c = pcc::row_reduce16(fg[j].c, add);
+            fg[j].x = pcc::row_reduce16(fg[j].x, add);
+            fg[j].y = pcc::row_reduce16(fg[j].y, add);
+            fg[j].z = pcc::row_reduce16(fg[j].z, add);
+        }
     }
     if (cl == 0) {
 #pragma unroll
         for (int j = 0; j < kFineQ; j++) {
             red[0][cs][og * kFineOG + quad * kFineQ + j] = s0[j];
             if (NW == 2) red[1][cs][og * kFineOG + quad * kFineQ + j] = s1[j];
-        }
-    }
-}
-
-template <int MODE, int CH>
+            if (FG) {
+                red[NW + 0][cs][og * kFineOG + quad * kFineQ + j] = fg[j].c;
+                red[NW + 1][cs][og * kFineOG + quad * kFineQ + j] = fg[j].x;
+                red[NW + 2][cs][og * kFineOG + quad * kFineQ + j] = fg[j].y;
+                red[NW + 3][cs][og * kFineOG + quad * kFineQ + j] = fg[j].z;
+            }
+        }
+    }
+}
+
+template <int MODE, int CH, bool FG = false>
 __global__ __launch_bounds__(64 * kFineS, MODE == PH_CA ? 4 : 8) void am_fine_kernel(PhaseArgs a) {
     constexpr int T = 64 * kFineS;
     constexpr int NW = (MODE == PH_CA) ? 2 : 1;
+    static_assert(!FG || MODE == PH_CA, "first-cloud sums: pass C only");
     constexpr bool W0_CONST = (MODE == PH_A);
     constexpr int NBLK = CH / kBox;
     static_assert(kFineGroups * NBLK == T, "one (owner group, candidate block) box test per thread");
     static_assert(kFineOG == kBox && kFineOG * kFineQ == 64, "a wave = 16 candidates x 4 owner quads");
     __shared__ __attribute__((aligned(16))) float lds_c[(3 + NW) * CH];
-    __shared__ float red[NW][2][64];
+    __shared__ float red[NW + (FG ? 4 : 0)][2][64];
     __shared__ unsigned char items[kFineGroups][NBLK];
     __shared__ unsigned char need[NBLK];
     __shared__ int wave_cnt[kFineS];
@@ -583,6 +700,16 @@
         const int oe = max(own_e, 0);
         if (MODE != PH_A && !a.first) pre_rem = a.remain[(size_t)smp * a.remain_stride + oe];
         if (MODE == PH_CA || MODE == PH_C) pre_ratio = a.ratio_in[(size_t)smp * a.ratio_stride + oe];
+    }
+    __shared__ float fg_park[FG ? 4 : 1][64];
+    FgSums fg[kFineQ];
+    if (FG) {
+        if (tid < 64) {
+            const FgOld v = fg_fetch(a.fg_grad + (size_t)smp * 3 * a.own_n4, a.fg_cost + (size_t)smp * a.n_own, max(own_e, 0), a.first);
+            fg_park[0][tid] = v.c; fg_park[1][tid] = v.x; fg_park[2][tid] = v.y; fg_park[3][tid] = v.z;
+        }
+#pragma unroll
+        for (int j = 0; j < kFineQ; j++) fg[j] = {0.f, 0.f, 0.f, 0.f};
     }
     const int tg = tid / NBLK, tb = tid - tg * NBLK;
     float4 glo, ghi;
@@ -630,11 +757,17 @@
             }
         }
         __syncthreads();
-        fine_walk<NW>(rows, items[og], wave_cnt[2 * og] + wave_cnt[2 * og + 1], cs, cl, c0, c1, own, s0, s1);
-    }
-    fine_reduce<NW>(s0, s1, red, cs, cl, og, quad);
+        fine_walk<NW, FG>(rows, items[og], wave_cnt[2 * og] + wave_cnt[2 * og + 1], cs, cl, c0, c1, own, s0, s1, fg);
+    }
+    fine_reduce<NW, FG>(s0, s1, red, cs, cl, og, quad, fg);
     __syncthreads();
     if (own_e < 0) return;
+    if (FG) {
+        const FgSums t = {red[NW + 0][0][tid] + red[NW + 0][1][tid], red[NW + 1][0][tid] + red[NW + 1][1][tid],
+                          red[NW + 2][0][tid] + red[NW + 2][1][tid], red[NW + 3][0][tid] + red[NW + 3][1][tid]};
+        const FgOld old = {fg_park[0][tid], fg_park[1][tid], fg_park[2][tid], fg_park[3][tid]};
+        fg_store(a.fg_grad + (size_t)smp * 3 * a.own_n4, a.fg_cost + (size_t)smp * a.n_own, own_e, old, pre_ratio, t);
+    }
     const float sum0 = red[0][0][tid] + red[0][1][tid];
     const float sum1 = NW == 2 ? red[NW - 1][0][tid] + red[NW - 1][1][tid] : 0.f;
     if (MODE == PH_A) {
@@ -979,6 +1112,7 @@
 
 template <int MODE, int R, int S, int G = 1>
 int launch_phase_rs(PhaseArgs a, int b, int var, hipStream_t st, const char *what) {
+    constexpr bool CMODE = MODE == PH_CA || MODE == PH_C;
     a.tiles = pcc::ceil_div(a.n_own, 64 * R / G);
     a.batch = b;
     const long long grid = (long long)b * a.tiles;
@@ -987,7 +1121,10 @@
         const bool skipping = (var == V_CLIST && (MODE == PH_CA || MODE == PH_C)) || (var == V_COWN && MODE == PH_B);
         pcc::ProfScope prof(phase_name<MODE>(a.level, skipping), st);
         const dim3 g((unsigned)grid), blk(64 * S);
-        if (var == V_CLIST && (MODE == PH_CA || MODE == PH_C))
+        if (CMODE && G == 1 && a.fg_grad) {
+            if (var == V_CLIST) hipLaunchKernelGGL((am_phase_kernel<CMODE ? MODE : PH_C, R, S, kClistCH, V_CLIST, 1, CMODE && G == 1>), g, blk, 0, st, a);
+            else hipLaunchKernelGGL((am_phase_kernel<CMODE ? MODE : PH_C, G == 1 ? R : 1, S, kPhCH, V_PLAIN, 1, CMODE && G == 1>), g, blk, 0, st, a);
+        } else if (var == V_CLIST && (MODE == PH_CA || MODE == PH_C))
             hipLaunchKernelGGL((am_phase_kernel<(MODE == PH_CA || MODE == PH_C) ? MODE : PH_C, R, S, kClistCH, V_CLIST>), g, blk, 0, st, a);
         else if (var == V_COWN && MODE == PH_B)
             hipLaunchKernelGGL((am_phase_kernel<PH_B, (G > 1 ? 1 : R), S, kPhCH, V_COWN, G>), g, blk, 0, st, a);
@@ -1004,7 +1141,8 @@
     if (grid > 0x7fffffffLL) return pcc::invalid("approxmatch: grid too large");
     {
         pcc::ProfScope prof(phase_name<MODE>(a.level, true), st);
-        hipLaunchKernelGGL((am_fine_kernel<(MODE == PH_C ? PH_CA : MODE), kPhCH>), dim3((unsigned)grid), dim3(64 * kFineS), 0, st, a);
+        if (MODE == PH_CA && a.fg_grad) hipLaunchKernelGGL((am_fine_kernel<PH_CA, kPhCH, true>), dim3((unsigned)grid), dim3(64 * kFineS), 0, st, a);
+        else hipLaunchKernelGGL((am_fine_kernel<(MODE == PH_C ? PH_CA : MODE), kPhCH>), dim3((unsigned)grid), dim3(64 * kFineS), 0, st, a);
     }
     return pcc::check_launch(what);
 }
@@ -1030,9 +1168,10 @@
     int b;
     int col_blocks, row_tiles;
     bool grad;
+    bool first;
     size_t total;
-    WsLayout(int b_, int n_, int m_, int col_blocks_ = 0, int row_tiles_ = 0, bool grad_ = false)
-        : AmDims(n_, m_), b(b_), col_blocks(col_blocks_), row_tiles(row_tiles_), grad(grad_) {
+    WsLayout(int b_, int n_, int m_, int col_blocks_ = 0, int row_tiles_ = 0, bool grad_ = false, bool first_ = false)
+        : AmDims(n_, m_), b(b_), col_blocks(col_blocks_), row_tiles(row_tiles_), grad(grad_), first(first_) {
         WsView unused;
         total = carve(0, 0, unused);
     }
@@ -1071,6 +1210,8 @@
         sec(v.pair_cost, (size_t)col_blocks * row_tiles);
         sec(v.part1, grad ? (size_t)row_tiles * n4 * 3 : 0);
         sec(v.part2, grad ? (size_t)col_blocks * m4 * 3 : 0);
+        sec(v.fg_grad, first ? 3 * (size_t)n4 : 0);
+        sec(v.fg_cost, first ? (size_t)n : 0);
         return o;
     }
 };
@@ -1129,6 +1270,7 @@
 }
 int launch_fine_resident(const Sched &sc, int bc, hipStream_t st) {
     if (!sc.skip || !sc.live_cnt || !sc.live_mask || !resident_enabled()) return -1;
+    if (sc.fg_grad) return -1;
     if (sc.n > kFpCH || sc.m > kFpCH || sc.n < 1 || sc.m < 1) return -1;
     const int tiles = pcc::ceil_div(std::max(sc.n, sc.m), 64);
     FinePersistArgs a{};
@@ -1170,6 +1312,7 @@
     sc.lc = lc;
     sc.clist = v.clist; sc.clist_cnt = v.clist_cnt;
     if (sc.skip) { sc.live_cnt = v.live_cnt; sc.live_mask = v.live_mask; }
+    if (L.first) { sc.fg_grad = v.fg_grad; sc.fg_cost = v.fg_cost; }
     return sc;
 }
 
@@ -1293,8 +1436,9 @@
                              float *cost, float *grad1, float *grad2, hipStream_t st,
                              const pcc::ChamferOut *chamfer = nullptr) {
     const bool grad = grad1 && grad2;
-    const int col_blocks = pcc::ceil_div(n, 64 * kPairQ), row_tiles = pcc::ceil_div(m, kPairRT);
-    const WsLayout L(b, n, m, col_blocks, row_tiles, grad);
+    const bool first = grad1 && !grad2;
+    const int col_blocks = first ? 0 : pcc::ceil_div(n, 64 * kPairQ), row_tiles = first ? 0 : pcc::ceil_div(m, kPairRT);
+    const WsLayout L(b, n, m, col_blocks, row_tiles, grad, first);
     pcc::WsBlock ws(st);
     if (int rc = ws.alloc(L.total, "workspace allocation failed")) return rc;
     char *base = static_cast<char *>(ws.p);
@@ -1371,7 +1515,7 @@
     hipStream_t st = static_cast<hipStream_t>(stream);
     if (n == 0 || m == 0) return zero_fill_empty(b, n, m, cost, grad1, grad2, st, "match_cost: memset failed");
     if (!xyz1 || !xyz2) return pcc::invalid("match_cost: null pointer");
-    if ((grad1 == nullptr) != (grad2 == nullptr)) return pcc::invalid("match_cost: grad1 and grad2 go together");
+    if (!grad1 && grad2) return pcc::invalid("match_cost: grad2 needs grad1 (grad1 alone, both, or neither)");
     return match_cost_implicit_impl(b, n, m, xyz1, xyz2, grad_cost, cost, grad1, grad2, st);
 }
 
diff --git a/pointcloudcounterfactual_amd/csrc/approxmatch.hpp b/pointcloudcounterfactual_amd/csrc/approxmatch.hpp
--- a/pointcloudcounterfactual_amd/csrc/approxmatch.hpp
+++ b/pointcloudcounterfactual_amd/csrc/approxmatch.hpp
@@ -79,6 +79,7 @@
     unsigned *live_mask;
     float4 *aos1, *aos2;
     float *pair_cost, *part1, *part2;
+    float *fg_grad, *fg_cost;
 };
 
 int sort_clouds(const AmDims &L, const WsView &v, int bc, const float *xyz1, const float *xyz2, bool aos, hipStream_t st);
diff --git a/pointcloudcounterfactual_amd/csrc/chamfer.hip b/pointcloudcounterfactual_amd/csrc/chamfer.hip
--- a/pointcloudcounterfactual_amd/csrc/chamfer.hip
+++ b/pointcloudcounterfactual_amd/csrc/chamfer.hip
@@ -381,7 +381,7 @@
     if (b > 65535) return pcc::invalid("chamfer_emd: batch too large");
     if (!xyz1 || !xyz2 || !chamfer_loss || !dist1 || !idx1 || !dist2 || !idx2 || !emd_cost)
         return pcc::invalid("chamfer_emd: null pointer");
-    if ((emd_grad1 == nullptr) != (emd_grad2 == nullptr)) return pcc::invalid("chamfer_emd: emd_grad1 and emd_grad2 go together");
+    if (!emd_grad1 && emd_grad2) return pcc::invalid("chamfer_emd: emd_grad2 needs emd_grad1 (emd_grad1 alone, both, or neither)");
     const pcc::ChamferOut ch{mean, chamfer_loss, dist1, dist2, idx1, idx2};
     return pcc::match_cost_with_chamfer(b, n, m, xyz1, xyz2, emd_cost, emd_grad1, emd_grad2,
                                         static_cast<hipStream_t>(stream), ch);
diff --git a/pointcloudcounterfactual_amd/losses.py b/pointcloudcounterfactual_amd/losses.py
--- a/pointcloudcounterfactual_amd/losses.py
+++ b/pointcloudcounterfactual_amd/losses.py
@@ -41,9 +41,9 @@
         ctx.mode = mode
         if mode == 'implicit':
             with_grad = bool(ctx.needs_input_grad[0] or ctx.needs_input_grad[1])
-            out = backend.MatchCostImplicit(set1, set2, with_grad)
+            out = backend.MatchCostImplicit(set1, set2, with_grad, grad2=bool(ctx.needs_input_grad[1]))
             if with_grad:
-                ctx.save_for_backward(out[1], out[2])
+                ctx.save_for_backward(*(g for g in out[1:] if g is not None))
             return out[0]
         ctx.save_for_backward(set1, set2)
         if mode == 'fused':
@@ -60,7 +60,7 @@
     def backward(ctx: Any, *grad_outputs: Any) -> tuple[torch.Tensor, torch.Tensor]:
         grad_output = grad_outputs[0]
         if ctx.mode == 'implicit':
-            grad1, grad2 = ctx.saved_tensors
+            grad1, grad2 = ctx.saved_tensors if ctx.needs_input_grad[1] else (ctx.saved_tensors[0], None)
             scale = grad_output.unsqueeze(1).unsqueeze(2)
             return (grad1 * scale if ctx.needs_input_grad[0] else None,
                     grad2 * scale if ctx.needs_input_grad[1] else None)
@@ -111,15 +111,16 @@
     def forward(ctx: Any, *args: Any, **kwargs: Any) -> Any:
         t1, t2, mean = args
         with_grad = bool(ctx.needs_input_grad[0] or ctx.needs_input_grad[1])
-        out = backend.ChamferEMD(t1, t2, bool(mean), with_grad)
+        out = backend.ChamferEMD(t1, t2, bool(mean), with_grad, grad2=bool(ctx.needs_input_grad[1]))
         if with_grad:
-            ctx.save_for_backward(t1, t2, out[1], out[2], out[4], out[5])
+            ctx.save_for_backward(t1, t2, out[1], out[2], *(g for g in out[4:6] if g is not None))
         ctx.mean = bool(mean)
         return out[0], out[3]
 
     @staticmethod
     def backward(ctx: Any, *grad_outputs: Any) -> Any:
-        t1, t2, idx1, idx2, e1, e2 = ctx.saved_tensors
+        t1, t2, idx1, idx2, e1, *rest = ctx.saved_tensors
+        e2 = rest[0] if rest else None
         gc, ge = grad_outputs
         gc = gc if gc.dtype == torch.float32 else gc.float()
         ge = ge if ge.dtype == torch.float32 else ge.float()
```

New measurement: 76580 clouds/s, median of 6. 1.05x the previous value.
